# westi024/RadTxfr

Measured on AMD Instinct MI355X. Metric: wavenumber*layer points/s (32-layer TUD, 500-6000 cm^-1 @ 0.001 cm^-1), higher is better.
Workload: dtype f32; 1 GPU; C3: 32-layer TUD (tau,Lu,Ld) StandardAtmosphere rows 1-32, 500-6000 cm^-1 @ 0.001 cm^-1; n_wavenumbers=5500000, n_layers=32, n_lines=100000, n_angles=30, line_table=synthetic HITRAN-format H2O+CO2, seed 20261005, parallelism=wavenumber-sharded x1, pipelines_per_gpu=3

## Files before the change

### include/radtxfr_hip.h

```cpp
#ifndef RADTXFR_HIP_H
#define RADTXFR_HIP_H

#include <stdint.h>

#ifdef __cplusplus
extern "C" {
#endif

#define RTX_VERSION 100

typedef struct rtx_grid {
  double xmin;
  double xmax;
  double step;
  int64_t n_total;
  int64_t offset;
  int64_t n;
} rtx_grid;

int rtx_version(void);
const char* rtx_last_error(void);
int rtx_device_info(char* name_h, int len, int* n_cu_h);

typedef struct rtx_lines rtx_lines;
// ... 40 lines not shown
                       const double* mass_h, double dil_air, double dil_self, double omega_wing, double omega_wing_hw,
                       double intensity_threshold, double scale, int profile, void* stream);

#define RTX_MAX_DILUENTS 8
int rtx_line_prep_mix(rtx_prep* prep, const rtx_lines* lines, const rtx_grid* grid, int n_layers, const double* T_h,
                      const double* p_atm_h, const double* qratio_h, const double* weight_h, const double* mass_h,
                      int n_dil, const int32_t* dil_h, const double* frac_h, double omega_wing, double omega_wing_hw,
                      double intensity_threshold, double scale, int profile, void* stream);
int rtx_line_prep_axis_mix(rtx_prep* prep, const rtx_lines* lines, const double* X_h, int64_t nx, int n_layers,
                           const double* T_h, const double* p_atm_h, const double* qratio_h, const double* weight_h,
                           const double* mass_h, int n_dil, const int32_t* dil_h, const double* frac_h, double omega_wing,
                           double omega_wing_hw, double intensity_threshold, double scale, int profile, void* stream);

int rtx_voigt_tile_points(void);
int rtx_voigt_sum(const rtx_prep* prep, const rtx_grid* grid, int n_layers, float* out_f32,
                  double* out_f64, int64_t ld, void* stream);
int rtx_voigt_sum_axis(const rtx_prep* prep, int n_layers, float* out_f32, double* out_f64, int64_t ld, void* stream);

int rtx_line_prep_dt(rtx_prep* prep, const rtx_lines* lines, const rtx_grid* grid, int n_layers, const double* T_h,
                     const double* p_atm_h, const double* qratio_h, const double* weight_h, const double* mass_h,
                     const double* dlnsw_h, double dil_air, double dil_self, double omega_wing, double omega_wing_hw,
                     double intensity_threshold, double scale, void* stream);
int rtx_voigt_sum_dt(const rtx_prep* prep, const rtx_grid* grid, int n_layers, float* out_f32, double* out_f64,
                     int64_t ld, void* stream);

int rtx_planck(const rtx_grid* grid, const double* X, int64_t nx, const double* T, int64_t nT,
               int wavelength, double* out, void* stream);

int rtx_brightness_temperature(const double* X, int64_t nx, const double* L, int64_t m,
                               int wavelength, double bad_value, double* T_out, void* stream);
int rtx_bt2l(const double* X, int64_t nx, const double* T, int64_t m, int wavelength,
             double bad_value, double* L_out, void* stream);

int rtx_tud(const float* OD, int64_t ld, const rtx_grid* grid, int n_layers, const double* T_h,
            int n_alt, const uint8_t* mask_h, int n_mu, const double* mu_h, int n_down,
            int n_angle, int return_od, float* tau, float* Lu, float* Ld, float* Ld_angles,
            int64_t ld_out, void* stream);
#define RTX_TUD_OD_NONNEG 1u
int rtx_tud_opts(const float* OD, int64_t ld, const rtx_grid* grid, int n_layers, const double* T_h,
                 int n_alt, const uint8_t* mask_h, int n_mu, const double* mu_h, int n_down,
                 int n_angle, int return_od, float* tau, float* Lu, float* Ld, float* Ld_angles,
                 int64_t ld_out, void* stream, unsigned flags);

int rtx_tud_jacobian(const float* OD, const float* OD_plus, const float* OD_minus, int64_t ld, double fd_step,
                     const float* K, int n_spec, const float* tau, int64_t ld_tau, const rtx_grid* grid,
                     int n_layers, const double* T_h, int n_alt, const uint8_t* mask_h, double mu, int n_down,
                     int n_angle, int return_od, const int32_t* layers_h, int n_lay, int t_pos, float* J,
                     int64_t ld_J, void* stream);
int rtx_tud_vjp(const float* OD, const float* OD_plus, const float* OD_minus, int64_t ld, double fd_step,
                const float* K, int n_spec, const float* tau, int64_t ld_tau, const rtx_grid* grid, int n_layers,
                const double* T_h, int n_alt, const uint8_t* mask_h, double mu, int n_down, int n_angle,
                int return_od, const int32_t* layers_h, int n_lay, int t_pos, const float* G_tau,
                const float* G_Lu, const float* G_Ld, int64_t ld_G, int n_vec, double* out, void* stream);
int rtx_tud_vjp_max_vectors(void);
int rtx_tud_jacobian_dod(const float* OD, const float* dOD_dT, int64_t ld, const float* K, int n_spec, const float* tau,
                         int64_t ld_tau, const rtx_grid* grid, int n_layers, const double* T_h, int n_alt,
                         const uint8_t* mask_h, double mu, int n_down, int n_angle, int return_od,
                         const int32_t* layers_h, int n_lay, int t_pos, float* J, int64_t ld_J, void* stream);
int rtx_tud_vjp_dod(const float* OD, const float* dOD_dT, int64_t ld, const float* K, int n_spec, const float* tau,
                    int64_t ld_tau, const rtx_grid* grid, int n_layers, const double* T_h, int n_alt,
                    const uint8_t* mask_h, double mu, int n_down, int n_angle, int return_od, const int32_t* layers_h,
                    int n_lay, int t_pos, const float* G_tau, const float* G_Lu, const float* G_Ld, int64_t ld_G,
                    int n_vec, double* out, void* stream);
int rtx_tud_jvp(const float* OD, const float* OD_plus, const float* OD_minus, int64_t ld, double fd_step,
                const float* K, int n_spec, const float* tau, int64_t ld_tau, const rtx_grid* grid, int n_layers,
                const double* T_h, int n_alt, const uint8_t* mask_h, double mu, int n_down, int n_angle,
                int return_od, int t_pos, const double* V_h, int n_vec, float* d_tau, float* d_Lu, float* d_Ld,
                int64_t ld_out, void* stream);
int rtx_tud_jvp_dod(const float* OD, const float* dOD_dT, int64_t ld, const float* K, int n_spec, const float* tau,
                    int64_t ld_tau, const rtx_grid* grid, int n_layers, const double* T_h, int n_alt,
                    const uint8_t* mask_h, double mu, int n_down, int n_angle, int return_od, int t_pos,
                    const double* V_h, int n_vec, float* d_tau, float* d_Lu, float* d_Ld, int64_t ld_out, void* stream);
int rtx_tud_jvp_max_vectors(void);
int rtx_tud_gtable_size(void);
int rtx_tud_gtable(int n_angle, double* table_h, double* g0_h);

int rtx_compute_tud(rtx_prep* prep, const rtx_lines* lines, const rtx_grid* grid, int n_layers,
                    const double* T_h, const double* p_atm_h, const double* qratio_h,
                    const double* weight_h, const double* mass_h, double dil_air, double dil_self,
                    double omega_wing, double omega_wing_hw, double intensity_threshold, int n_alt,
                    const uint8_t* mask_h, int n_mu, const double* mu_h, int n_down, int n_angle,
                    int return_od, float* OD, int64_t ld_od, float* tau, float* Lu, float* Ld,
                    int64_t ld_out, void* stream);

int rtx_apparent_radiance(const double* X, int64_t nX, const float* emis, int64_t nE,
                          const double* Ts, int64_t nA, const float* tau, const float* La,
                          const float* Ld, const double* dT, int64_t nT, float* L, float* Ls,
                          void* stream);

int rtx_ils(int kind, const rtx_grid* grid, const double* X, int64_t nx, const float* Y,
            int64_t nS, int64_t ldY, int nB, const double* centre, const double* sigma,
            float* Y_out, void* stream);

int rtx_srf_apply(const rtx_grid* grid, const double* X, int64_t nx, const float* Y, int64_t nS,
                  int64_t ldY, int nB, const int32_t* knot_start, const double* knot_x,
                  const float* knot_r, float* Y_out, float* wsum_out, void* stream);
int rtx_srf_chunk_points(void);
int rtx_srf_max_knots(void);

int rtx_interp_knots(const rtx_grid* grid, const double* X, int64_t nx, const double* Xk,
                     int64_t nk, const float* F, int64_t nS, float* out, void* stream);

int rtx_band_moments(int kind, const rtx_grid* grid, const float* tau, const float* La,
                     const float* Ld, double Ts, const double* Xk, int64_t nk, int nB,
                     const double* centre, const double* sigma, float* N_out, float* C_out,
                     float* M_out, int32_t* jrange_out, void* stream);
int rtx_band_mix(const float* N, const float* C, const float* M, const int32_t* jrange, int nB,
                 int64_t nk, const float* E, int64_t nE, float* out, void* stream);

int rtx_srf_moments(const rtx_grid* grid, const float* tau, const float* La, const float* Ld,
                    const double* Ts_h, int nT, const double* Xk, int64_t nk, int nB,
                    const int32_t* knot_start, const double* knot_x, const float* knot_r,
                    float* N_out, float* C_out, float* M_out, int32_t* jrange_out, void* stream);
int rtx_srf_moments_max_temps(void);

int rtx_srf_radiance_vjp(const rtx_grid* grid, const float* tau, const float* La, const float* Ld,
                         const double* Ts_h, int nT, const double* Xk, int64_t nk, int nB,
                         const int32_t* knot_start, const double* knot_x, const float* knot_r,
                         const float* E, int64_t nE, const float* g, float* G_tau, float* G_La,
                         float* G_Ld, double* dTs, double* dE, void* stream);
int rtx_srf_norms(const rtx_grid* grid, int nB, const int32_t* knot_start, const double* knot_x,
                  const float* knot_r, float* N_out, void* stream);

int rtx_srf_radiance_jvp(const rtx_grid* grid, const float* tau, const float* Ld, const float* d_tau,
                         const float* d_La, const float* d_Ld, int64_t ld_d, const double* Ts_h,
                         const double* dTs_h, int nT, const double* Xk, int64_t nk, int nB,
                         const int32_t* knot_start, const double* knot_x, const float* knot_r,
                         const float* N, const float* M, const int32_t* jrange, const float* E,
                         const float* dE, int64_t nE, int n_vec, float* dL, void* stream);
int rtx_srf_radiance_jvp_max_vectors(void);
int rtx_srf_radiance_jvp_max_temps(void);

int rtx_band_basis_moments(int kind, const rtx_grid* grid, const float* tau, const float* La,
                           const float* Ld, const double* Xk, int64_t nk, int nB,
                           const double* centre, const double* sigma, int Q,
                           const float* basis_coef_h, double node_span, float* N_out,
                           float* C_out, float* MLd_out, float* MB_out, int32_t* jrange_out,
                           void* stream);
int rtx_band_mix_stacked(const float* M, const int32_t* jrange, int nB, int n_stack, int64_t nk,
                         const float* E, int64_t nE, float* tab, void* stream);
int rtx_pixel_cube(int nB, int Q, const double* centre, const double* sigma, double node_span,
                   const float* s_node_h, const float* N, const float* C, const float* tab,
                   int nEnd, int64_t nPix, int nMix, const int32_t* kidx, const float* frac,
                   const double* Tpix, float* cube, void* stream);

int rtx_srf_cube_max_nodes(void);
int rtx_srf_cube_tables(const float* M, const int32_t* jrange, int nB, int Q, int64_t nk,
                        const float* E, int64_t nEnd, float* tab, void* stream);
int rtx_srf_pixel_cube(int nB, int Q, const double* T_node_h, const float* N, const float* C,
                       const float* tab, int nEnd, int64_t nPix, int nMix, const int32_t* kidx,
                       const float* frac, const double* Tpix, float* cube, void* stream);

int rtx_srf_pixel_cube_vjp(int nB, int Q, const double* T_node_h, const float* N, const float* tab,
                           int nEnd, int64_t nPix, int nMix, const int32_t* kidx, const float* frac,
                           const double* Tpix, const float* g, double* dT, double* dfrac, float* gL,
                           void* stream, unsigned flags);

int rtx_sdvoigt_sum(const rtx_prep* prep, const rtx_grid* grid, int n_layers, float* out_f32,
                    double* out_f64, int64_t ld, void* stream);

#define RTX_LS_PCQSDHC 0
#define RTX_LS_LORENTZ 1
#define RTX_LS_DOPPLER 2
#define RTX_CPF_HUM1_WEI 0
#define RTX_CPF_CPF3 1
int rtx_profile_eval(int kind, int64_t n_lines, const double* params, const double* sg, int64_t n,
// ... 75 lines not shown
```

### radtxfr_amd/_lib.py

```python
import ctypes as C
import os

_HERE = os.path.dirname(os.path.abspath(__file__))
LIB_PATH = os.environ.get("RADTXFR_LIB") or os.path.join(_HERE, "libradtxfr_hip.so")


class RtxGrid(C.Structure):
    _fields_ = [("xmin", C.c_double), ("xmax", C.c_double), ("step", C.c_double),
                ("n_total", C.c_int64), ("offset", C.c_int64), ("n", C.c_int64)]


_vp, _i64, _i32, _dbl = C.c_void_p, C.c_int64, C.c_int, C.c_double
_pd = C.POINTER(C.c_double)
_gp = C.POINTER(RtxGrid)

PROTOTYPES = {
    "rtx_version": (_i32, []),
    "rtx_last_error": (C.c_char_p, []),
    "rtx_device_info": (_i32, [C.c_char_p, _i32, C.POINTER(_i32)]),
    "rtx_lines_create": (_i32, [_i64, _i32] + [_vp] * 10 + [_vp, C.POINTER(_vp)]),
    "rtx_lines_free": (_i32, [_vp]),
    "rtx_lines_count": (_i64, [_vp]),
    "rtx_prep_create": (_i32, [_vp, _i32, _i64, C.POINTER(_vp)]),
    "rtx_prep_free": (_i32, [_vp]),
    "rtx_line_prep": (_i32, [_vp, _vp, _gp, _i32, _vp, _vp, _vp, _vp, _vp, _dbl, _dbl, _dbl, _dbl, _dbl, _dbl, _vp]),
    "rtx_line_prep_profile": (_i32, [_vp, _vp, _gp, _i32, _vp, _vp, _vp, _vp, _vp, _dbl, _dbl, _dbl, _dbl, _dbl, _dbl, _i32, _vp]),
    "rtx_prep_split_bound": (_i64, [_vp]),
    "rtx_line_prep_window": (_i32, [_vp, _vp, _gp, _i32, _vp, _vp, _vp, _vp, _vp, _vp, _dbl, _dbl, _dbl, _dbl, _dbl, _dbl, _i32, _vp]),
    "rtx_line_prep_axis": (_i32, [_vp, _vp, _vp, _i64, _i32, _vp, _vp, _vp, _vp, _vp, _dbl, _dbl, _dbl, _dbl, _dbl, _dbl, _i32, _vp]),
    "rtx_voigt_sum": (_i32, [_vp, _gp, _i32, _vp, _vp, _i64, _vp]),
    "rtx_voigt_sum_axis": (_i32, [_vp, _i32, _vp, _vp, _i64, _vp]),
    "rtx_sdvoigt_sum": (_i32, [_vp, _gp, _i32, _vp, _vp, _i64, _vp]),
    "rtx_lines_set_sd": (_i32, [_vp, _vp, _vp]),
    "rtx_lines_set_deltap_self": (_i32, [_vp, _vp]),
    "rtx_lines_set_broadeners": (_i32, [_vp, _i32, _vp, _vp, _vp, _vp, _vp]),
    "rtx_line_prep_mix": (_i32, [_vp, _vp, _gp, _i32, _vp, _vp, _vp, _vp, _vp, _i32, _vp, _vp, _dbl, _dbl, _dbl, _dbl, _i32, _vp]),
    "rtx_line_prep_axis_mix": (_i32, [_vp, _vp, _vp, _i64, _i32, _vp, _vp, _vp, _vp, _vp, _i32, _vp, _vp, _dbl, _dbl, _dbl, _dbl,
                                       _i32, _vp]),
    "rtx_voigt_tile_points": (_i32, []),
    "rtx_planck": (_i32, [_gp, _vp, _i64, _vp, _i64, _i32, _vp, _vp]),
    "rtx_tud": (_i32, [_vp, _i64, _gp, _i32, _vp, _i32, _vp, _i32, _vp, _i32, _i32, _i32, _vp, _vp, _vp, _vp, _i64, _vp]),
    "rtx_tud_opts": (_i32, [_vp, _i64, _gp, _i32, _vp, _i32, _vp, _i32, _vp, _i32, _i32, _i32, _vp, _vp, _vp, _vp, _i64, _vp, C.c_uint]),
    "rtx_tud_jacobian": (_i32, [_vp, _vp, _vp, _i64, _dbl, _vp, _i32, _vp, _i64, _gp, _i32, _vp, _i32, _vp, _dbl, _i32, _i32,
                                 _i32, _vp, _i32, _i32, _vp, _i64, _vp]),
    "rtx_tud_vjp": (_i32, [_vp, _vp, _vp, _i64, _dbl, _vp, _i32, _vp, _i64, _gp, _i32, _vp, _i32, _vp, _dbl, _i32, _i32,
                            _i32, _vp, _i32, _i32, _vp, _vp, _vp, _i64, _i32, _vp, _vp]),
    "rtx_tud_vjp_max_vectors": (_i32, []),
    "rtx_line_prep_dt": (_i32, [_vp, _vp, _gp, _i32, _vp, _vp, _vp, _vp, _vp, _vp, _dbl, _dbl, _dbl, _dbl, _dbl, _dbl, _vp]),
    "rtx_voigt_sum_dt": (_i32, [_vp, _gp, _i32, _vp, _vp, _i64, _vp]),
    "rtx_tud_jacobian_dod": (_i32, [_vp, _vp, _i64, _vp, _i32, _vp, _i64, _gp, _i32, _vp, _i32, _vp, _dbl, _i32, _i32,
                                     _i32, _vp, _i32, _i32, _vp, _i64, _vp]),
    "rtx_tud_vjp_dod": (_i32, [_vp, _vp, _i64, _vp, _i32, _vp, _i64, _gp, _i32, _vp, _i32, _vp, _dbl, _i32, _i32,
                                _i32, _vp, _i32, _i32, _vp, _vp, _vp, _i64, _i32, _vp, _vp]),
    "rtx_tud_jvp": (_i32, [_vp, _vp, _vp, _i64, _dbl, _vp, _i32, _vp, _i64, _gp, _i32, _vp, _i32, _vp, _dbl, _i32, _i32,
                            _i32, _i32, _vp, _i32, _vp, _vp, _vp, _i64, _vp]),
    "rtx_tud_jvp_dod": (_i32, [_vp, _vp, _i64, _vp, _i32, _vp, _i64, _gp, _i32, _vp, _i32, _vp, _dbl, _i32, _i32,
                                _i32, _i32, _vp, _i32, _vp, _vp, _vp, _i64, _vp]),
    "rtx_tud_jvp_max_vectors": (_i32, []),
    "rtx_tud_gtable_size": (_i32, []),
    "rtx_tud_gtable": (_i32, [_i32, _vp, _vp]),
    "rtx_compute_tud": (_i32, [_vp, _vp, _gp, _i32, _vp, _vp, _vp, _vp, _vp, _dbl, _dbl, _dbl, _dbl, _dbl, _i32, _vp, _i32, _vp,
                                _i32, _i32, _i32, _vp, _i64, _vp, _vp, _vp, _i64, _vp]),
    "rtx_apparent_radiance": (_i32, [_vp, _i64, _vp, _i64, _vp, _i64, _vp, _vp, _vp, _vp, _i64, _vp, _vp, _vp]),
    "rtx_ils": (_i32, [_i32, _gp, _vp, _i64, _vp, _i64, _i64, _i32, _vp, _vp, _vp, _vp]),
    "rtx_srf_apply": (_i32, [_gp, _vp, _i64, _vp, _i64, _i64, _i32, _vp, _vp, _vp, _vp, _vp, _vp]),
    "rtx_srf_chunk_points": (_i32, []),
    "rtx_srf_max_knots": (_i32, []),
    "rtx_srf_moments": (_i32, [_gp, _vp, _vp, _vp, _vp, _i32, _vp, _i64, _i32, _vp, _vp, _vp, _vp, _vp, _vp, _vp, _vp]),
    "rtx_srf_moments_max_temps": (_i32, []),
    "rtx_srf_radiance_vjp": (_i32, [_gp, _vp, _vp, _vp, _vp, _i32, _vp, _i64, _i32, _vp, _vp, _vp, _vp, _i64, _vp, _vp, _vp, _vp,
                                     _vp, _vp, _vp]),
    "rtx_srf_norms": (_i32, [_gp, _i32, _vp, _vp, _vp, _vp, _vp]),
    "rtx_srf_radiance_jvp": (_i32, [_gp, _vp, _vp, _vp, _vp, _vp, _i64, _vp, _vp, _i32, _vp, _i64, _i32, _vp, _vp, _vp, _vp, _vp,
                                     _vp, _vp, _vp, _i64, _i32, _vp, _vp]),
    "rtx_srf_radiance_jvp_max_vectors": (_i32, []),
    "rtx_srf_radiance_jvp_max_temps": (_i32, []),
    "rtx_interp_knots": (_i32, [_gp, _vp, _i64, _vp, _i64, _vp, _i64, _vp, _vp]),
    "rtx_band_moments": (_i32, [_i32, _gp, _vp, _vp, _vp, _dbl, _vp, _i64, _i32, _vp, _vp, _vp, _vp, _vp, _vp, _vp]),
    "rtx_band_mix": (_i32, [_vp, _vp, _vp, _vp, _i32, _i64, _vp, _i64, _vp, _vp]),
    "rtx_band_basis_moments": (_i32, [_i32, _gp, _vp, _vp, _vp, _vp, _i64, _i32, _vp, _vp, _i32, _vp, _dbl,
                                      _vp, _vp, _vp, _vp, _vp, _vp]),
    "rtx_band_mix_stacked": (_i32, [_vp, _vp, _i32, _i32, _i64, _vp, _i64, _vp, _vp]),
    "rtx_pixel_cube": (_i32, [_i32, _i32, _vp, _vp, _dbl, _vp, _vp, _vp, _vp, _i32, _i64, _i32, _vp, _vp, _vp, _vp, _vp]),
    "rtx_srf_cube_max_nodes": (_i32, []),
    "rtx_srf_cube_tables": (_i32, [_vp, _vp, _i32, _i32, _i64, _vp, _i64, _vp, _vp]),
    "rtx_srf_pixel_cube": (_i32, [_i32, _i32, _vp, _vp, _vp, _vp, _i32, _i64, _i32, _vp, _vp, _vp, _vp, _vp]),
    "rtx_srf_pixel_cube_vjp": (_i32, [_i32, _i32, _vp, _vp, _vp, _i32, _i64, _i32, _vp, _vp, _vp, _vp, _vp, _vp, _vp, _vp, C.c_uint]),
    "rtx_fir_reflect": (_i32, [_vp, _i32, _i64, _i32, _i64, _vp, _i32, _i32, _vp, _i64, _vp]),
    "rtx_cubic_resample": (_i32, [_vp, _i64, _i32, _i64, _dbl, _dbl, _vp, _i64, _vp, _i64, _vp]),
    "rtx_cubic_end": (_i32, [_vp, _i64, _i32, _i64, _i32, _i32, _i32, _vp, _vp, _i64, _vp, _i64, _vp]),
    "rtx_cubic_resample_unchecked": (_i32, [_vp, _i64, _i32, _i64, _dbl, _dbl, _vp, _i64, _vp, _i64, _vp]),
    "rtx_hapi_spectrum": (_i32, [_i32, _gp, _vp, _vp, _i32, _i32, _i64, _i64, _dbl, _dbl, _vp, _i64, _vp]),
    "rtx_fir_same": (_i32, [_vp, _i32, _i64, _i32, _i64, _vp, _i64, _dbl, _i64, _i64, _vp, _i64, _vp]),
    "rtx_profile_eval": (_i32, [_i32, _i64, _vp, _vp, _i64, _vp, _vp, _i64, _vp]),
    "rtx_profile_sum": (_i32, [_i64, _vp, _vp, _vp, _vp, _i64, _vp, _vp]),
    "rtx_cpf_eval": (_i32, [_i32, _vp, _vp, _i64, _vp, _vp, _vp]),
    "rtx_lines_set_ht": (_i32, [_vp, _i32, _vp, _vp]),
    "rtx_ht_create": (_i32, [_i64, _i32, _i64, C.POINTER(_vp)]),
    "rtx_ht_free": (_i32, [_vp]),
    "rtx_ht_prep": (_i32, [_vp, _vp, _vp, _i64, _i32, _vp, _vp, _vp, _vp, _vp, _i32, _vp, _vp, _dbl, _dbl, _dbl, _dbl, _vp]),
    "rtx_ht_sum": (_i32, [_vp, _i32, _vp, _vp, _i64, _vp]),
    "rtx_ht_params": (_i32, [_vp, _i32, _vp, _vp, _vp, _vp]),
    "rtx_fir_tile_points": (_i32, []),
    "rtx_fir_chunk_taps": (_i32, []),
    "rtx_brightness_temperature": (_i32, [_vp, _i64, _vp, _i64, _i32, _dbl, _vp, _vp]),
    "rtx_bt2l": (_i32, [_vp, _i64, _vp, _i64, _i32, _dbl, _vp, _vp]),
    "rtx_xs_lut_create": (_i32, [_i32, _i64, _i64, C.POINTER(_vp)]),
    "rtx_xs_lut_free": (_i32, [_vp]),
    "rtx_xs_lut_bytes": (_i64, [_vp]),
    "rtx_xs_lut_set_rows": (_i32, [_vp, _i64, _i64, _vp, _vp]),
    "rtx_xs_lut_get_rows": (_i32, [_vp, _i64, _i64, _vp, _vp]),
    "rtx_xs_od": (_i32, [_vp, _i64, _i64, _i32, _vp, _vp, _vp, _i64, _vp]),
    "rtx_xs_tile_points": (_i32, []),
    "rtx_xs_od_d": (_i32, [_vp, _i64, _i64, _i32, _vp, _vp, _i32, _vp, _vp, _vp, _vp, _i64, _vp, C.c_uint]),
    "rtx_continuum_add": (_i32, [_gp, _i32, _vp, _i32, _vp, _vp, _vp, _vp, _i64, _vp, _i64, _vp, C.c_uint]),
    "rtx_continuum_tile_points": (_i32, []),
    "rtx_continuum_add_d": (_i32, [_gp, _i32, _vp, _i32, _vp, _vp, _vp, _vp, _vp, _vp, _i64, _vp, _i32, _vp, _vp, _i64, _vp,
                                   C.c_uint]),
    "rtx_comm_init_all": (_i32, [_i32, _vp, _i32, C.POINTER(_vp)]),
    "rtx_comm_backend": (_i32, [_vp]),
    "rtx_allgather": (_i32, [_vp, _vp, _vp, _i64, _vp]),
    "rtx_comm_destroy": (_i32, [_vp]),
}

_lib = None


class RtxError(RuntimeError):
    pass


def load():
    global _lib
    if _lib is not None:
        return _lib
    if not os.path.exists(LIB_PATH):
        raise RtxError(
            f"{LIB_PATH} not found: build it with `python -c 'import __graft_entry__ as g; g.build()'` "
            f"or `make -C radtxfr_amd/csrc` (hipcc --offload-arch=gfx950). There is no CPU fallback.")
    import torch
    lib = C.CDLL(LIB_PATH)
    for name, (res, args) in PROTOTYPES.items():
        try:
            fn = getattr(lib, name)
        except AttributeError as e:
# ... 19 lines not shown
```

### radtxfr_amd/csrc/rtx_common.h

```cpp
#pragma once
#include <hip/hip_runtime.h>
#include <math.h>
#include <stdint.h>
#include <stdio.h>

#include <vector>

#include "../../include/radtxfr_hip.h"
#include "rtx_devmem.h"

void rtx_set_error(const char* fmt, ...);
#define RTX_FAIL(...)          \
  do {                         \
    rtx_set_error(__VA_ARGS__); \
    return 1;                  \
  } while (0)
#define RTX_HIP(call)                                                                        \
  do {                                                                                       \
    hipError_t e_ = (call);                                                                  \
    if (e_ != hipSuccess) RTX_FAIL("%s:%d %s -> %s", __FILE__, __LINE__, #call, hipGetErrorString(e_)); \
  } while (0)
#define RTX_LAUNCH_CHECK()                                                                   \
  do {                                                                                       \
    hipError_t e_ = hipGetLastError();                                                       \
// ... 69 lines not shown
  double nu, cte, Gam0, Shift0, Gam2, WS;
  double inv_Gam2, csqrtY;
};

struct __attribute__((aligned(16))) LineRecDT64 {
  double alpha;
  double sx;
  double gy;
  double h;
};
struct __attribute__((aligned(16))) LineRecDT {
  float alpha, sx, yp, h;
  float Ap;
  float yh;
  float y2;
  float y;
};

struct rtx_lines {
  long long n = 0;
  int n_species = 0;
  DevBuf<double> nu, sw, elower, gamma_air, gamma_self, n_air, n_self, delta_air, deltap_air, delta_self;
  DevBuf<double> sd_air, sd_self;
  DevBuf<double> deltap_self;
  DevBuf<double> zn;
  DevBuf<int> species;
  std::vector<double> nu_host;
  double ga_max = 0.0, gs_max = 0.0, n_lo = 1e300, n_hi = -1e300;
  double na_lo = 1e300, na_hi = -1e300, ns_lo = 1e300, ns_hi = -1e300;
  int n_extra = 0;
  DevBuf<double> x_gamma, x_n, x_delta, x_deltap, x_sd;
  std::vector<double> x_gmax, x_nlo, x_nhi;
  DevBuf<double> ht_data;
  DevBuf<const double*> ht_ptr;
};

#ifndef RTX_SPLIT_PART
#define RTX_SPLIT_PART 256
#endif
#ifndef RTX_SPLIT_MIN
#define RTX_SPLIT_MIN 768
#endif
struct __attribute__((aligned(16))) SplitItem {
  int tile, k;
  int lo, hi;
  int part;
  int extra;
  int pad0, pad1;
};

struct rtx_prep {
  long long n_lines = 0;
  int max_layers = 0;
  int n_layers = 0;
  DevBuf<LineRec> rec;
  DevBuf<LineRec64> rec64;
  DevBuf<int> ic;
  DevBuf<int2> win;
  DevBuf<int> maxhw;
  int* smally = nullptr;
  int* n_items = nullptr;
  DevBuf<int2> ranges;
  DevBuf<LineRecSD> recsd;
  long long max_tiles = 0;
  DevBuf<double> env;
  double scale = 0.0;
  DevBuf<SplitItem> items;
  DevBuf<float> part_ws;
  long long split_bound = 0;
  double split_W = 0.0;
  double split_xmin = 0.0, split_step = 0.0;
  long long split_off = 0, split_n = 0;
  int split_layers = 0;
  const void* split_lines = nullptr;
  DevBuf<double> X;
  long long nx = 0;
  int axis = 0;
  DevBuf<double> twin;
  DevBuf<double> frac;
  DevBuf<LineRecDT> drec;
  DevBuf<LineRecDT64> drec64;
  DevBuf<double> dlnsw;
  int dT = 0;
};
```

### radtxfr_amd/csrc/rtx_tud.hip

```cpp
#include <math.h>
#include <stdlib.h>
#include <string.h>

#include <map>
#include <mutex>
#include <vector>

#include "rtx_tud_common.h"

struct PlanckArgs {
  GridDev g;
  const double* X;
  long long nx, nT;
  const double* T;
  int wavelength;
  double* out;
};

__global__ __launch_bounds__(256) void planck_kernel(PlanckArgs a) {
  const long long total = a.nx * a.nT;
  for (long long e = (long long)blockIdx.x * blockDim.x + threadIdx.x; e < total; e += (long long)gridDim.x * blockDim.x) {
    const long long i = e / a.nT, j = e - i * a.nT;
    double X = a.X ? a.X[i] : grid_x(a.g, a.g.offset + i);
    const double T = a.T[j];
// ... 47 lines not shown
    double X = a.X[i];
    const double v = a.in[e];
    double r;
    bool bad;
    if (a.inverse) {
      double L = v;
      if (a.wavelength) {
        X = X * 1e-6;  L = L * 1e4;
        r = RT_C2 / (X * log(1.0 + RT_C1 / (pow(X, 5.0) * L)));
      } else {
        X = X * 100.0;  L = L * 1e-4;
        r = RT_C2 * X / log(RT_C1 * (X * X * X) / L + 1.0);
      }
      bad = !isfinite(L) || (L <= 0.0);
    } else {
      const double T = v;
      if (a.wavelength) {
        X = X * 1e-6;
        r = RT_C1 / (pow(X, 5.0) * (exp(RT_C2 / (X * T)) - 1.0));
        r *= 1e-4;
      } else {
        X = X * 100.0;
        r = RT_C1 * (X * X * X) / (exp(RT_C2 * X / T) - 1.0);
        r *= 1e4;
      }
      bad = !isfinite(r) || (T <= 0.0);
    }
    a.out[e] = bad ? a.bad : r;
  }
}

static int launch_bt(const double* X, int64_t nx, const double* in, int64_t m, int wavelength, int inverse, double bad,
                     double* out, void* stream) {
  if (nx < 0 || m < 0) RTX_FAIL("negative size");
  if (nx == 0 || m == 0) return 0;
  if (!X || !in || !out) RTX_FAIL("a required pointer is NULL");
  BtArgs a;
  a.X = X; a.nx = nx; a.m = m; a.in = in; a.wavelength = wavelength; a.inverse = inverse; a.bad = bad; a.out = out;
  long long blocks = (nx * m + 255) / 256;
  if (blocks > 256 * 32) blocks = 256 * 32;
  hipLaunchKernelGGL(bt_kernel, dim3((unsigned)blocks), dim3(256), 0, (hipStream_t)stream, a);
  RTX_LAUNCH_CHECK();
  return 0;
}

extern "C" int rtx_brightness_temperature(const double* X, int64_t nx, const double* L, int64_t m, int wavelength,
                                          double bad_value, double* T_out, void* stream) {
  return launch_bt(X, nx, L, m, wavelength, 1, bad_value, T_out, stream);
}

extern "C" int rtx_bt2l(const double* X, int64_t nx, const double* T, int64_t m, int wavelength, double bad_value,
                        double* L_out, void* stream) {
  return launch_bt(X, nx, T, m, wavelength, 0, bad_value, L_out, stream);
}

#define TUD_MAX_LAYERS 128
#define TUD_MAX_ANGLES 128
#define TUD_MAX_ALT 16
#define TUD_MAX_MU 8

struct TudArgs {
  const float* OD;
  long long ld, ld_out;
  GridDev g;
  int n_layers, n_alt, n_mu, n_down, n_ang, return_od;
  float* tau;
  float* Lu;
  float* Ld;
  float* Ld_ang;
  int n_ang_real;
  float inv_wsum;
  double c2l2e_over_T[TUD_MAX_LAYERS];
  double c2l2e_over_Tmax, c2l2e_over_Tmin;
  float ang_c[TUD_MAX_ANGLES];
  float ang_w[TUD_MAX_ANGLES];
  float ang_cmin, ang_cmax;
  float mu_c[TUD_MAX_MU];
  float mu[TUD_MAX_MU];
  unsigned int mask[TUD_MAX_ALT][TUD_MAX_LAYERS / 32];
  int count[TUD_MAX_ALT];
  const double* gtab;
  double g0;
  int skip;
};

#define TUD_OPAQUE_Y 26.0f

__device__ __forceinline__ double readlane_f64(double v, int lane) {
  const int lo = __builtin_amdgcn_readlane(__double2loint(v), lane), hi = __builtin_amdgcn_readlane(__double2hiint(v), lane);
  return __hiloint2double(hi, lo);
}
struct TudLane {
  bool live;
  long long i;
  const float* __restrict__ od_col;
  double x, c1x3;
  double ct_a, ct_b;
  __device__ __forceinline__ explicit TudLane(const TudArgs& a) {
    const long long i_raw = (long long)blockIdx.x * blockDim.x + threadIdx.x;
    live = i_raw < a.g.n;
    i = live ? i_raw : a.g.n - 1;
    od_col = a.OD + i;
    x = grid_x(a.g, a.g.offset + i);
    const double x100 = x * 100.0;
    c1x3 = RT_C1 * (x100 * x100 * x100) * 1e4;
  }
  __device__ __forceinline__ void layer_consts(const TudArgs& a) {
    const int lane_id = threadIdx.x & 63, nL = a.n_layers;
    ct_a = a.c2l2e_over_T[lane_id < nL ? lane_id : 0];
    ct_b = a.c2l2e_over_T[lane_id + 64 < nL ? lane_id + 64 : 0];
  }
  __device__ __forceinline__ double c2l2e_of(int k) const { return readlane_f64(k < 64 ? ct_a : ct_b, k & 63); }
  __device__ __forceinline__ float planck(int k) const { return planck_f32(c1x3, x, c2l2e_of(k)); }
};

struct LayerMask {
  unsigned w0, w1, w2, w3;
  __device__ __forceinline__ bool bit(int k) const {
    const unsigned w = k < 32 ? w0 : k < 64 ? w1 : k < 96 ? w2 : w3;
    return (w >> (k & 31)) & 1u;
  }
};
__device__ __forceinline__ LayerMask layer_mask(const TudArgs& a, int ia) {
  return LayerMask{a.mask[ia][0], a.mask[ia][1], a.mask[ia][2], a.mask[ia][3]};
}

__device__ __forceinline__ float up_step(float Lu, float B, float y) {
  return (y > -TUD_THIN_Y) ? fmaf(em_thin(y), B - Lu, Lu) : fmaf(__builtin_amdgcn_exp2f(y), Lu - B, B);
}

__device__ __forceinline__ float opaque_y(const TudArgs& a, const TudLane& l) {
  const float b_hot = planck_f32(l.c1x3, l.x, a.c2l2e_over_Tmax), b_cold = planck_f32(l.c1x3, l.x, a.c2l2e_over_Tmin);
  const float r = __builtin_amdgcn_logf(b_hot / b_cold);
  return (b_cold > 0.f && r == r && r < 1e30f) ? TUD_OPAQUE_Y + 1.0f + fmaxf(r, 0.f) : 3.0e38f;
}

#ifndef TUD_STAGE
#define TUD_STAGE 4
#endif
#ifndef TUD_ABLATE
#define TUD_ABLATE 0
#endif
#ifndef TUD_ILP
#define TUD_ILP 8
#endif
#define TUD_COL_LAYERS 36
template <int NA, bool COL>
__global__ __launch_bounds__(256) void tud_kernel(TudArgs a) {
  extern __shared__ float s_od[];
  float (*s_stage)[256] = reinterpret_cast<float (*)[256]>(s_od);
  TudLane ln(a);
  const bool live = ln.live;
  const long long i = ln.i;
  const int nL = a.n_layers;
  const float* __restrict__ od_col = ln.od_col;
  if (COL) {
    float* dst = &s_stage[0][threadIdx.x & ~63u];
    for (int k = 0; k < nL; ++k)
      __builtin_amdgcn_global_load_lds((const __attribute__((address_space(1))) void*)(od_col + (size_t)k * a.ld),
                                       (__attribute__((address_space(3))) void*)(dst + k * 256), 4, 0, 0);
  }
  const double x = ln.x, c1x3 = ln.c1x3;
  if (COL) asm volatile("s_waitcnt vmcnt(0)" ::: "memory");
  ln.layer_consts(a);
  auto od_at = [&](int k) -> float { return COL ? s_stage[k][threadIdx.x] : od_col[(size_t)k * a.ld]; };
  auto planck_of = [&](int k) -> float { return COL ? planck_f32(c1x3, x, readlane_f64(ln.ct_a, k & 63)) : ln.planck(k); };
// ... 241 lines not shown
}

struct PlanckNodes {
  float c0, c1, c2;
  float c0b, c1b, c2b;
  float t;
};
__device__ __forceinline__ PlanckNodes planck_nodes_setup(const TudArgs& a, const TudLane& l) {
  PlanckNodes P;
  const double ct_a = l.ct_a, ct_b = l.ct_b;
  const int nL = a.n_layers;
  const long long i0w = (long long)blockIdx.x * blockDim.x + (threadIdx.x & ~63u);
  const float t1 = 32.0f / 63.0f;
  float b[3], bb[3];
#pragma unroll
  for (int n = 0; n < 3; ++n) {
    const double xn = grid_x(a.g, a.g.offset + i0w + (n == 0 ? 0 : n == 1 ? 32 : 63));
    const double x100 = xn * 100.0;
    const double c1x3 = RT_C1 * (x100 * x100 * x100) * 1e4;
    b[n] = planck_f32(c1x3, xn, ct_a);
    bb[n] = nL > 64 ? planck_f32(c1x3, xn, ct_b) : 0.f;
  }
  {
    const float d01 = (b[1] - b[0]) / t1, d12 = (b[2] - b[1]) / (1.0f - t1);
    P.c2 = d12 - d01; P.c1 = d01 - P.c2 * t1; P.c0 = b[0];
  }
  {
    const float d01 = (bb[1] - bb[0]) / t1, d12 = (bb[2] - bb[1]) / (1.0f - t1);
    P.c2b = d12 - d01; P.c1b = d01 - P.c2b * t1; P.c0b = bb[0];
  }
  P.t = (float)(threadIdx.x & 63) * (1.0f / 63.0f);
  return P;
}
__device__ __forceinline__ float planck_nodes_eval(const PlanckNodes& P, bool hi, int lane) {
  const float c0 = __int_as_float(__builtin_amdgcn_readlane(__float_as_int(hi ? P.c0b : P.c0), lane));
  const float c1 = __int_as_float(__builtin_amdgcn_readlane(__float_as_int(hi ? P.c1b : P.c1), lane));
  const float c2 = __int_as_float(__builtin_amdgcn_readlane(__float_as_int(hi ? P.c2b : P.c2), lane));
  return fmaf(fmaf(c2, P.t, c1), P.t, c0);
}
__device__ __forceinline__ float planck_nodes_eval(const PlanckNodes& P, int k) {
  if (k < 64) return planck_nodes_eval(P, false, k);
  return planck_nodes_eval(P, true, k - 64);
}

__device__ __forceinline__ void tudg_load(double* s_g, const TudArgs& a) {
  for (int t = threadIdx.x; t < TUDG_NINT * 4; t += 256) reinterpret_cast<double2*>(s_g)[t] = reinterpret_cast<const double2*>(a.gtab)[t];
}

struct TudDown {
  double S, g_prev, g_floor;
  float acc;
  bool live;
  __device__ __forceinline__ TudDown(const double* s_g, const TudArgs& a, const TudLane& l) {
    S = 0.0;
    g_prev = tudg_eval(s_g, 0.0);
    acc = 0.f;
    g_floor = a.g0 * (double)__builtin_amdgcn_exp2f(-fminf(opaque_y(a, l), 120.0f));
    live = a.n_down > 0;
  }
  __device__ __forceinline__ TudDown(const double* s_g, const TudArgs& a, float y_opq) {
    S = 0.0;
    g_prev = tudg_eval(s_g, 0.0);
    acc = 0.f;
    g_floor = a.g0 * (double)__builtin_amdgcn_exp2f(-fminf(y_opq, 120.0f));
    live = a.n_down > 0;
  }
  __device__ __forceinline__ void step(const double* s_g, float od, float B) {
    S += (double)od;
    const double g = tudg_eval(s_g, S);
    acc = fmaf(B, (float)(g_prev - g), acc);
    g_prev = g;
    if (__ballot(g > g_floor) == 0ull) live = false;
  }
  __device__ __forceinline__ float result(const TudArgs& a) const {
    return (S != S) ? __builtin_nanf("") : acc * a.inv_wsum;
  }
};

#define TUD_SKIP_SCAN (3 * TUD_STAGE)
#define TUD_SKIP_BOTTOM TUD_STAGE
#define TUD_SKIP_MARGIN 8.0f
#define TUD_SKIP_TAU0 151.0f

template <bool PN, bool SKIP>
__global__ __launch_bounds__(256) void tud_g_kernel(TudArgs a) {
  static_assert(PN || !SKIP, "the look at the top is written for the Planck-node instantiation");
  __shared__ double s_g[TUDG_NINT * 8];
  __shared__ float s_stage[(SKIP ? 2 : 1) * TUD_STAGE][256];
  tudg_load(s_g, a);
  TudLane ln(a);
  const int nL = a.n_layers;
  const float* __restrict__ od_col = ln.od_col;
  float nxt[TUD_STAGE];
#pragma unroll
  for (int t = 0; t < TUD_STAGE; ++t) nxt[t] = od_col[(size_t)(t < nL ? t : nL - 1) * a.ld];
  ln.layer_consts(a);
  const LayerMask mask0 = layer_mask(a, 0);
  PlanckNodes PNd;
  if (PN) PNd = planck_nodes_setup(a, ln);
  __syncthreads();

  for (int p = 1; p < a.n_alt * a.n_mu; ++p) {
    const int ia = p / a.n_mu, im = p - ia * a.n_mu;
    const int cnt = a.count[ia];
    const float c = a.mu_c[im];
    float s = 0.f, Lu = 0.f;
    for (int k = 0; k < nL; ++k) {
      const float od = ln.od_col[(size_t)k * a.ld];
      if ((a.mask[ia][k >> 5] >> (k & 31)) & 1u) s += od;
      if (k < cnt) Lu = up_step(Lu, PN ? planck_nodes_eval(PNd, k) : ln.planck(k), od * c);
    }
    if (ln.live) {
      const size_t o = (size_t)p * (size_t)a.ld_out + (size_t)ln.i;
      a.tau[o] = a.return_od ? s * a.mu[im] : __builtin_amdgcn_exp2f(s * c);
      a.Lu[o] = Lu;
    }
  }

  const int nd = a.n_down, cnt0 = a.count[0];
  const float c0 = a.mu_c[0];
  float s0 = 0.f, Lu0 = 0.f;
  const float y_opq = SKIP ? opaque_y(a, ln) : 0.f;
  TudDown down = SKIP ? TudDown(s_g, a, y_opq) : TudDown(s_g, a, ln);
  bool skip_armed = SKIP;
  const unsigned long long m_lo = (unsigned long long)mask0.w0 | ((unsigned long long)mask0.w1 << 32);
  const unsigned long long m_hi = (unsigned long long)mask0.w2 | ((unsigned long long)mask0.w3 << 32);
  const size_t bump = (size_t)TUD_STAGE * (size_t)a.ld;
  const float y_up = y_opq + TUD_SKIP_MARGIN;
  const int k_top = (cnt0 - 1) & ~(TUD_STAGE - 1);
  int k_look = -1;
  const float* pf[TUD_STAGE];
#pragma unroll
  for (int t = 0; t < TUD_STAGE; ++t) pf[t] = od_col + (size_t)(TUD_STAGE + t) * (size_t)a.ld;
  for (int kc = 0; kc < nL; kc += TUD_STAGE) {
#pragma unroll
    for (int t = 0; t < TUD_STAGE; ++t) s_stage[t][threadIdx.x] = nxt[t];
    if (kc + 2 * TUD_STAGE <= nL) {
#pragma unroll
      for (int t = 0; t < TUD_STAGE; ++t) nxt[t] = *pf[t];
    } else {
#pragma unroll
      for (int t = 0; t < TUD_STAGE; ++t)
        if (kc + TUD_STAGE + t < nL) nxt[t] = *pf[t];
    }
#pragma unroll
    for (int t = 0; t < TUD_STAGE; ++t) pf[t] += bump;
    const int k_hi = kc + TUD_STAGE < nL ? kc + TUD_STAGE : nL;
    if (PN && k_hi == kc + TUD_STAGE && k_hi <= cnt0 && k_hi <= nd) {
      const unsigned mchunk = (unsigned)((kc < 64 ? m_lo : m_hi) >> (kc & 63));
      const bool hi_set = kc >= 64;
#pragma unroll
      for (int t = 0; t < TUD_STAGE; ++t) {
        const float od = s_stage[t][threadIdx.x];
        if ((mchunk >> t) & 1u) s0 += od;
        const float B = planck_nodes_eval(PNd, hi_set, (kc & 63) + t);
        Lu0 = up_step(Lu0, B, od * c0);
        if (down.live) down.step(s_g, od, B);
      }
      if (SKIP && !down.live) {
        if (skip_armed) {
          skip_armed = false;
          if (k_hi <= TUD_SKIP_BOTTOM && k_hi + TUD_STAGE <= k_top) { k_look = k_hi; break; }
        }
      }
    } else {
      for (int k = kc; k < k_hi; ++k) {
        const float od = s_stage[k - kc][threadIdx.x];
        if (mask0.bit(k)) s0 += od;
        const bool up = k < cnt0, dn = down.live && k < nd;
        if (!up && !dn) continue;
        const float B = PN ? planck_nodes_eval(PNd, k) : ln.planck(k);
        if (up) Lu0 = up_step(Lu0, B, od * c0);
        if (dn) down.step(s_g, od, B);
      }
      if (SKIP && skip_armed && !(down.live && k_hi < nd)) {
        skip_armed = false;
        if (k_hi <= TUD_SKIP_BOTTOM && k_hi + TUD_STAGE <= k_top) { k_look = k_hi; break; }
      }
    }
  }
  if (SKIP && k_look >= 0) {
    int kc = k_look;
    unsigned tid_top = threadIdx.x;
    asm volatile("" : "+v"(tid_top));
    const long long i_top = (long long)blockIdx.x * blockDim.x + tid_top;
    const float* __restrict__ od_top = a.OD + (i_top < a.g.n ? i_top : a.g.n - 1);
    constexpr int NC = TUD_SKIP_SCAN / TUD_STAGE;
    const float ac0 = -c0;
    const int k_deep = k_top - (TUD_SKIP_SCAN - TUD_STAGE);
    const int k_scan = k_deep > kc + TUD_STAGE ? k_deep : kc + TUD_STAGE;
    static_assert(NC == 3, "the look at the top is laid out for three chunks");
    float v0[TUD_STAGE];
#pragma unroll
    for (int t = 0; t < TUD_STAGE; ++t) v0[t] = od_top[(size_t)(k_top + t < cnt0 ? k_top + t : cnt0 - 1) * (size_t)a.ld];
    {
      float* dst = &s_stage[0][threadIdx.x & ~63u];
      const int n_dma = k_top - 2 * TUD_STAGE >= k_scan ? 2 * TUD_STAGE : k_top - TUD_STAGE >= k_scan ? TUD_STAGE : 0;
      const float* pc = od_top + (size_t)(k_top - n_dma) * (size_t)a.ld;
      float* d = dst + (n_dma == TUD_STAGE ? TUD_STAGE * 256 : 0);
#pragma unroll 1
      for (int j = 0; j < n_dma; ++j) {
        __builtin_amdgcn_global_load_lds((const __attribute__((address_space(1))) void*)pc, (__attribute__((address_space(3))) void*)d, 4, 0, 0);
        pc += a.ld;
        d += 256;
      }
    }
    asm volatile("s_waitcnt vmcnt(0)" ::: "memory");
    float s_top = 0.f;
#pragma unroll
    for (int t = TUD_STAGE - 1; t >= 0; --t)
      if (k_top + t < cnt0) s_top += v0[t];
    int k_res = -1;
    if (__ballot(s_top * ac0 >= y_up) == ~0ull) k_res = k_top;
#pragma unroll 1
    for (int c = 1; c < NC && k_res < 0 && k_top - c * TUD_STAGE >= k_scan; ++c) {
      const int slot = c == 1 ? TUD_STAGE : 0;
#pragma unroll
      for (int t = TUD_STAGE - 1; t >= 0; --t) s_top += s_stage[slot + t][threadIdx.x];
      if (__ballot(s_top * ac0 >= y_up) == ~0ull) k_res = k_top - c * TUD_STAGE;
    }
    if (k_res < 0) {
#pragma unroll
      for (int t = 0; t < TUD_STAGE; ++t) pf[t] = od_top + (size_t)(kc + TUD_STAGE + t) * (size_t)a.ld;
      for (; kc < cnt0; kc += TUD_STAGE) {
#pragma unroll
        for (int t = 0; t < TUD_STAGE; ++t) s_stage[t][threadIdx.x] = nxt[t];
#pragma unroll
        for (int t = 0; t < TUD_STAGE; ++t)
          if (kc + TUD_STAGE + t < cnt0) nxt[t] = *pf[t];
#pragma unroll
        for (int t = 0; t < TUD_STAGE; ++t) pf[t] += bump;
        if (kc + TUD_STAGE <= cnt0) {
          const bool hi_set = kc >= 64;
#pragma unroll
          for (int t = 0; t < TUD_STAGE; ++t) {
            const float od = s_stage[t][threadIdx.x];
            s0 += od;
            Lu0 = up_step(Lu0, planck_nodes_eval(PNd, hi_set, (kc & 63) + t), od * c0);
          }
        } else {
          for (int k = kc; k < cnt0; ++k) {
            const float od = s_stage[k - kc][threadIdx.x];
            s0 += od;
            Lu0 = up_step(Lu0, planck_nodes_eval(PNd, k), od * c0);
          }
        }
      }
    } else {
    for (int km = kc; km < k_res; km += TUD_STAGE) {
      if (__ballot((s0 + s_top) * ac0 >= TUD_SKIP_TAU0) == ~0ull) break;
      float w[TUD_STAGE];
#pragma unroll
      for (int t = 0; t < TUD_STAGE; ++t) w[t] = od_top[(size_t)(km + t) * (size_t)a.ld];
#pragma unroll
      for (int t = 0; t < TUD_STAGE; ++t) s0 += w[t];
    }
#pragma unroll 1
    for (int kb = k_res; kb < k_top; kb += TUD_STAGE) {
      const int slot = kb == k_top - TUD_STAGE ? TUD_STAGE : 0;
#pragma unroll
      for (int t = 0; t < TUD_STAGE; ++t) {
        const float od = s_stage[slot + t][threadIdx.x];
        s0 += od;
        Lu0 = up_step(Lu0, planck_nodes_eval(PNd, kb + t), od * c0);
      }
    }
#pragma unroll
    for (int t = 0; t < TUD_STAGE; ++t) {
      if (k_top + t < cnt0) {
        s0 += v0[t];
        Lu0 = up_step(Lu0, planck_nodes_eval(PNd, k_top + t), v0[t] * c0);
      }
    }
    }
  }
  long long i_out = ln.i;
  bool live_out = ln.live;
  if (SKIP) {
    unsigned tid_out = threadIdx.x;
    asm volatile("" : "+v"(tid_out));
    i_out = (long long)blockIdx.x * blockDim.x + tid_out;
    live_out = i_out < a.g.n;
  }
  if (live_out) {
    a.tau[i_out] = a.return_od ? s0 * a.mu[0] : __builtin_amdgcn_exp2f(s0 * c0);
    a.Lu[i_out] = Lu0;
    a.Ld[i_out] = down.result(a);
  }
}

#ifndef TUDG_PB
#define TUDG_PB 3
#endif
template <int PB>
__global__ __launch_bounds__(256) void tud_g_pairs_kernel(TudArgs a) {
  __shared__ double s_g[TUDG_NINT * 8];
  __shared__ float s_stage[TUD_STAGE][256];
  tudg_load(s_g, a);
  TudLane ln(a);
  const int nL = a.n_layers;
  const float* __restrict__ od_col = ln.od_col;
  ln.layer_consts(a);
// ... 131 lines not shown
        s_run += od;
#pragma unroll
        for (int m = 0; m < NMU; ++m)
          if (NMU == 1 || m < n_mu) Lu[m] = up_step(Lu[m], B, od * cm[m]);
        if ((snap_chunk >> t) & 1u) snapshot(kc + t + 1);
        if (down.live) down.step(s_g, od, B);
      }
      continue;
    }
    for (int k = kc; k < k_hi; ++k) {
      const float od = s_stage[k - kc][threadIdx.x];
      const bool up = k < cnt_max, dn = down.live && k < nd;
      if (!up && !dn) continue;
      const float B = PN ? planck_nodes_eval(PNd, k) : ln.planck(k);
      if (up) {
        s_run += od;
#pragma unroll
        for (int m = 0; m < NMU; ++m)
          if (m < n_mu) Lu[m] = up_step(Lu[m], B, od * cm[m]);
        snapshot(k + 1);
      }
      if (dn) down.step(s_g, od, B);
    }
  }
  if (ln.live) a.Ld[ln.i] = down.result(a);
}

static void tudg_build(int n_angle, std::vector<double>& tab, double& g0_out) {
  const TudQuadrature quad = tud_quadrature(n_angle);
  std::vector<double> sec;
  for (int ii = 1; ii < n_angle; ++ii) sec.push_back(1.0 / cos(quad.th[ii]));
  auto G = [&](double S) { double r = 0.0; for (size_t q = 0; q < sec.size(); ++q) r += quad.w[q + 1] * exp(-S * sec[q]); return r; };
  constexpr int N = TUDG_DEG + 1;
  tab.assign((size_t)TUDG_NINT * 8, 0.0);
  for (int idx = 0; idx < TUDG_NINT; ++idx) {
    double lo, hi;
    if (idx < TUDG_NLOG) {
      union { int i; float f; } a0, a1;
      a0.i = (TUDG_BASE + idx) << (23 - TUDG_M);
      a1.i = (TUDG_BASE + idx + 1) << (23 - TUDG_M);
      lo = (double)a0.f - (double)TUDG_OFF;
      hi = (double)a1.f - (double)TUDG_OFF;
      if (lo < 0.0) lo = 0.0;
      if (hi > (double)TUDG_SWITCH) hi = (double)TUDG_SWITCH;
    } else {
      lo = (double)TUDG_SWITCH + 0.5 * (idx - TUDG_NLOG);
      hi = lo + 0.5;
    }
    const double mid = 0.5 * (lo + hi), hw = 0.5 * (hi - lo) * 1.002;
    double y[N], c[N];
    for (int k = 0; k < N; ++k) y[k] = G(mid + hw * cos(M_PI * (k + 0.5) / N));
    for (int j = 0; j < N; ++j) {
      double sacc = 0.0;
      for (int k = 0; k < N; ++k) sacc += y[k] * cos(M_PI * j * (k + 0.5) / N);
      c[j] = sacc * (j == 0 ? 1.0 : 2.0) / N;
    }
    double mono[N] = {0}, Tm[N] = {0}, Tc[N] = {0}, Tn[N];
    Tm[0] = 1.0;
    Tc[1] = 1.0;
    mono[0] += c[0];
    if (N > 1) mono[1] += c[1];
    for (int n = 2; n < N; ++n) {
      for (int d = 0; d < N; ++d) Tn[d] = (d > 0 ? 2.0 * Tc[d - 1] : 0.0) - Tm[d];
      for (int d = 0; d < N; ++d) { mono[d] += c[n] * Tn[d]; Tm[d] = Tc[d]; Tc[d] = Tn[d]; }
    }
    double* row = &tab[(size_t)idx * 8];
    row[0] = mid;
    double sc = 1.0;
    for (int d = 0; d < N; ++d) { row[1 + d] = mono[d] * sc; sc /= hw; }
  }
  g0_out = quad.wsum;
}

extern "C" int rtx_tud_gtable_size(void) { return TUDG_NINT * 8; }
extern "C" int rtx_tud_gtable(int n_angle, double* table_h, double* g0_h) {
  if (n_angle < 1 || n_angle > TUD_MAX_ANGLES - 32) RTX_FAIL("n_angle=%d outside [1,%d]", n_angle, TUD_MAX_ANGLES - 32);
  if (!table_h || !g0_h) RTX_FAIL("a required pointer is NULL");
  std::vector<double> tab;
  tudg_build(n_angle, tab, *g0_h);
  memcpy(table_h, tab.data(), tab.size() * sizeof(double));
  return 0;
}

static int tudg_table(int n_angle, DevTableCache<double>::Hit* out) {
  static DevTableCache<double>* const cache = new DevTableCache<double>(0);
  int dev = 0;
  RTX_HIP(hipGetDevice(&dev));
  return cache->get(dev, &n_angle, sizeof(n_angle), [&](std::vector<double>& tab) { double g0; tudg_build(n_angle, tab, g0); return 0; }, out);
}

static int tud_launch(void (*kernel)(TudArgs), const TudArgs& a, size_t lds_bytes, hipStream_t st) {
  hipLaunchKernelGGL(kernel, dim3((unsigned)((a.g.n + 255) / 256)), dim3(256), lds_bytes, st, a);
  RTX_LAUNCH_CHECK();
  return 0;
}

template <int NA>
static int launch_tud(TudArgs& a, int na, hipStream_t st) {
  const int na_pad = na == 0 ? NA : ((na + NA - 1) / NA) * NA;
  float cmin = (float)LOG2E, cmax = (float)LOG2E;
  for (int q = 0; q < na; ++q) { cmin = q == 0 ? -a.ang_c[q] : fminf(cmin, -a.ang_c[q]); cmax = q == 0 ? -a.ang_c[q] : fmaxf(cmax, -a.ang_c[q]); }
  for (int q = na; q < na_pad; ++q) { a.ang_c[q] = na > 0 ? a.ang_c[na - 1] : (float)(-LOG2E); a.ang_w[q] = 0.f; }
  a.ang_cmin = cmin; a.ang_cmax = cmax;
  a.n_ang = na_pad;
  if (a.n_layers <= TUD_COL_LAYERS) return tud_launch(tud_kernel<NA, true>, a, (size_t)a.n_layers * 256 * sizeof(float), st);
  return tud_launch(tud_kernel<NA, false>, a, (size_t)TUD_STAGE * 256 * sizeof(float), st);
}

extern "C" int rtx_tud_opts(const float* OD, int64_t ld, const rtx_grid* grid, int n_layers, const double* T_h, int n_alt,
                            const uint8_t* mask_h, int n_mu, const double* mu_h, int n_down, int n_angle, int return_od,
                            float* tau, float* Lu, float* Ld, float* Ld_angles, int64_t ld_out, void* stream, unsigned flags) {
  if (rtx_check_grid(grid)) return 1;
  if (flags & ~(unsigned)RTX_TUD_OD_NONNEG) RTX_FAIL("flags=0x%x: unknown bits", flags);
  if (!OD || !T_h || !mask_h || !mu_h || !tau || !Lu || !Ld) RTX_FAIL("a required pointer is NULL");
  if (n_layers < 1 || n_layers > TUD_MAX_LAYERS) RTX_FAIL("n_layers=%d outside [1,%d]", n_layers, TUD_MAX_LAYERS);
  if (n_alt < 1 || n_alt > TUD_MAX_ALT) RTX_FAIL("n_alt=%d outside [1,%d]", n_alt, TUD_MAX_ALT);
  if (n_mu < 1 || n_mu > TUD_MAX_MU) RTX_FAIL("n_mu=%d outside [1,%d]", n_mu, TUD_MAX_MU);
  if (n_angle < 1 || n_angle > TUD_MAX_ANGLES - 32) RTX_FAIL("n_angle=%d outside [1,%d]", n_angle, TUD_MAX_ANGLES - 32);
  if (n_down < 0 || n_down > n_layers) RTX_FAIL("n_down=%d outside [0,%d]", n_down, n_layers);
  if (ld < grid->n || ld_out < grid->n) RTX_FAIL("leading dimension smaller than the shard");
  if (grid->n == 0) return 0;
  TudArgs a;
  memset(&a, 0, sizeof(a));
  a.OD = OD; a.ld = ld; a.ld_out = ld_out; a.g = to_dev(grid);
  a.n_layers = n_layers; a.n_alt = n_alt; a.n_mu = n_mu; a.n_down = n_down; a.return_od = return_od;
  a.tau = tau; a.Lu = Lu; a.Ld = Ld; a.Ld_ang = Ld_angles;
  if (tud_layer_consts(T_h, n_layers, a.c2l2e_over_T)) return 1;
  double t_max = T_h[0], t_min = T_h[0];
  for (int k = 1; k < n_layers; ++k) {
    if (T_h[k] > t_max) t_max = T_h[k];
    if (T_h[k] < t_min) t_min = T_h[k];
  }
  a.c2l2e_over_Tmax = c2l2e_over(t_max);
  a.c2l2e_over_Tmin = c2l2e_over(t_min);
  for (int ia = 0; ia < n_alt; ++ia) {
    int c = 0;
    for (int k = 0; k < n_layers; ++k)
      if (mask_h[(size_t)ia * n_layers + k]) { a.mask[ia][k >> 5] |= 1u << (k & 31); ++c; }
    a.count[ia] = c;
  }
  for (int m = 0; m < n_mu; ++m) { a.mu[m] = (float)mu_h[m]; a.mu_c[m] = (float)(-LOG2E * mu_h[m]); }
  const TudQuadrature quad = tud_quadrature(n_angle);
  int na = 0;
  for (int ii = Ld_angles ? 0 : 1; ii < n_angle; ++ii) {
    a.ang_c[na] = (float)(-LOG2E / cos(quad.th[ii]));
    a.ang_w[na] = (float)quad.w[ii];
    ++na;
  }
  a.n_ang_real = na;
  a.inv_wsum = (float)(1.0 / quad.wsum);
  if (na == 0) a.inv_wsum = NAN;
  hipStream_t st = (hipStream_t)stream;
  static int force_streams = -1;
  if (force_streams < 0) { const char* e = getenv("RADTXFR_TUD_KERNEL"); force_streams = (e && !strcmp(e, "streams")) ? 1 : 0; }
  if (!Ld_angles && !force_streams) {
    DevTableCache<double>::Hit gt;
    if (tudg_table(n_angle, &gt)) return 1;
    a.gtab = gt.d; a.g0 = quad.wsum;
    bool prefix = true;
    for (int ia = 0; ia < n_alt && prefix; ++ia)
      for (int k = 0; k < n_layers; ++k)
        if ((mask_h[(size_t)ia * n_layers + k] != 0) != (k < a.count[ia])) { prefix = false; break; }
    const double nu_lo = grid->xmin;
    const bool pn = nu_lo > 0.0 && (4.0 / nu_lo + RT_C2 * 100.0 / t_min) * 63.0 * grid->step <= 7e-3;
    void (*kernel)(TudArgs);
    if (n_alt * n_mu == 1) {
      kernel = pn ? tud_g_kernel<true, false> : tud_g_kernel<false, false>;
      static int skip_on = -1;
      if (skip_on < 0) { const char* e = getenv("RADTXFR_TUD_SKIP"); skip_on = (e && !strcmp(e, "0")) ? 0 : 1; }
      a.skip = skip_on && (flags & RTX_TUD_OD_NONNEG) && !return_od && prefix && pn;
      if (a.skip) kernel = tud_g_kernel<true, true>;
    }
    else if (prefix && n_mu == 1) kernel = pn ? tud_g_snap_kernel<1, true> : tud_g_snap_kernel<1, false>;
    else if (prefix) kernel = pn ? tud_g_snap_kernel<TUD_MAX_MU, true> : tud_g_snap_kernel<TUD_MAX_MU, false>;
    else kernel = tud_g_pairs_kernel<TUDG_PB>;
    return tud_launch(kernel, a, 0, st);
  }
  if (na <= 4) return launch_tud<4>(a, na, st);
  if (na <= 8) return launch_tud<8>(a, na, st);
  if (na <= 16) return launch_tud<16>(a, na, st);
  if (na <= 24) return launch_tud<24>(a, na, st);
  if (na <= 29) return launch_tud<29>(a, na, st);
  return launch_tud<32>(a, na, st);
}

extern "C" int rtx_tud(const float* OD, int64_t ld, const rtx_grid* grid, int n_layers, const double* T_h, int n_alt,
                       const uint8_t* mask_h, int n_mu, const double* mu_h, int n_down, int n_angle, int return_od,
                       float* tau, float* Lu, float* Ld, float* Ld_angles, int64_t ld_out, void* stream) {
  return rtx_tud_opts(OD, ld, grid, n_layers, T_h, n_alt, mask_h, n_mu, mu_h, n_down, n_angle, return_od, tau, Lu, Ld, Ld_angles,
                      ld_out, stream, 0u);
}

extern "C" int rtx_compute_tud(rtx_prep* prep, const rtx_lines* lines, const rtx_grid* grid, int n_layers, const double* T_h,
                               const double* p_atm_h, const double* qratio_h, const double* weight_h, const double* mass_h,
                               double dil_air, double dil_self, double omega_wing, double omega_wing_hw,
                               double intensity_threshold, int n_alt, const uint8_t* mask_h, int n_mu, const double* mu_h,
                               int n_down, int n_angle, int return_od, float* OD, int64_t ld_od, float* tau, float* Lu,
                               float* Ld, int64_t ld_out, void* stream) {
  if (!OD) RTX_FAIL("OD workspace is NULL");
  if (rtx_line_prep_profile(prep, lines, grid, n_layers, T_h, p_atm_h, qratio_h, weight_h, mass_h, dil_air, dil_self, omega_wing,
                            omega_wing_hw, intensity_threshold, 1.0, RTX_PROFILE_VOIGT, stream))
    return 1;
  if (rtx_voigt_sum(prep, grid, n_layers, OD, nullptr, ld_od, stream)) return 1;
  auto nonneg = [](const double* v, long long n) {
    for (long long j = 0; j < n; ++j)
      if (!(v[j] >= 0.0 && v[j] <= 1.7976931348623157e308)) return false;
    return true;
  };
  const long long n_sl = (long long)lines->n_species * n_layers;
  const unsigned flags = nonneg(weight_h, n_sl) && nonneg(qratio_h, n_sl) && nonneg(T_h, n_layers) && nonneg(p_atm_h, n_layers)
                             ? RTX_TUD_OD_NONNEG : 0u;
  return rtx_tud_opts(OD, ld_od, grid, n_layers, T_h, n_alt, mask_h, n_mu, mu_h, n_down, n_angle, return_od, tau, Lu, Ld, nullptr,
                      ld_out, stream, flags);
}
```

### radtxfr_amd/csrc/rtx_voigt.hip

```cpp
#include <stdlib.h>
#include <string.h>

#include "rtx_common.h"

#include "rtx_voigt_math.h"

struct RangeArgs {
  const int* ic;
  const int* maxhw;
  const int2* win;
  long long n_lines;
  int n_tiles, tile, n_layers, n_steps;
  long long n;
  int2* ranges;
  SplitItem* items;
  int* n_items;
  long long items_cap;
};

#define RNG_G 16
__device__ __forceinline__ unsigned group_bits(unsigned long long b, int lane) { return (unsigned)(b >> (lane & 48)) & 0xffffu; }

template <bool STRICT>
__device__ __forceinline__ void bound_step(const int* __restrict__ ic, int& lo, int& hi, int v, int sub, int lane) {
  const unsigned width = (unsigned)(hi - lo);
  const int stride = (int)((width + RNG_G) / (unsigned)(RNG_G + 1));
  const long long pl = (long long)lo + (long long)(sub + 1) * stride - 1;
  const bool inside = width > 0 && pl < (long long)hi;
  const int p = inside ? (int)pl : lo;
  const bool pred = inside && (STRICT ? ic[p] < v : ic[p] <= v);
  const int c = __popc(group_bits(__ballot(pred), lane));
  if (width > 0) {
    const long long cap = (long long)lo + (long long)(c + 1) * stride - 1;
    if (c < RNG_G && cap < (long long)hi) hi = (int)cap;
    lo += c * stride;
  }
}

__global__ __launch_bounds__(256) void tile_ranges_kernel(RangeArgs a) {
  const int lane = threadIdx.x & 63, sub = lane & (RNG_G - 1);
  const int t = (int)((blockIdx.x * blockDim.x + threadIdx.x) / RNG_G);
  const int k = blockIdx.y;
  const bool live = t < a.n_tiles;
  const long long ia = (long long)t * a.tile;
  long long ib = ia + a.tile;
  if (ib > a.n) ib = a.n;
  const long long hw = a.maxhw[k];
  int l0 = 0, h0 = live ? (int)a.n_lines : 0, l1 = 0, h1 = h0;
  {
    const long long v0 = ia - hw, v1 = ib - 1 + hw;
    const int k0 = (int)(v0 < -2147483647LL ? -2147483647LL : v0), k1 = (int)(v1 > 2147483647LL ? 2147483647LL : v1);
    for (int it = 0; it < a.n_steps; ++it) {
      bound_step<true>(a.ic, l0, h0, k0, sub, lane);
      bound_step<false>(a.ic, l1, h1, k1, sub, lane);
    }
  }
  if (l1 < l0) l1 = l0;
  const int2* __restrict__ win = a.win + (size_t)k * (size_t)a.n_lines;
  long long first = l1, last = l1;
  {
    int base = l0, top = l1;
    bool done_f = base >= l1, done_b = done_f;
    while (__ballot(!done_f || !done_b)) {
      const int sf = base + sub, sb = top - 1 - sub;
      int2 wf = make_int2(0, 0), wb = wf;
      if (!done_f && sf < l1) wf = win[sf];
      if (!done_b && sb >= l0) wb = win[sb];
      const bool rf = (long long)wf.y > ia && (long long)wf.x < ib && wf.y > wf.x;
      const bool rb = (long long)wb.y > ia && (long long)wb.x < ib && wb.y > wb.x;
      const unsigned mf = group_bits(__ballot(rf), lane), mb = group_bits(__ballot(rb), lane);
      if (!done_f) {
        if (mf) { first = base + __builtin_ctz(mf); done_f = true; }
        else { base += RNG_G; done_f = base >= l1; }
      }
      if (!done_b) {
        if (mb) { last = top - __builtin_ctz(mb); done_b = true; }
        else { top -= RNG_G; done_b = top <= l0; }
      }
    }
    if (first >= l1) last = first = l1;
  }
  if (live && sub == 0) {
    const long long cnt = last - first;
    if (a.items && cnt > RTX_SPLIT_MIN) {
      const int extra = (int)((cnt - 1) / RTX_SPLIT_PART);
      const long long at = (long long)atomicAdd(a.n_items, extra);
      if (at + extra <= a.items_cap) {
        for (int p = 1; p <= extra; ++p) {
          SplitItem it;
          it.tile = t; it.k = k; it.part = p; it.extra = extra; it.pad0 = it.pad1 = 0;
          it.lo = (int)(first + (long long)p * RTX_SPLIT_PART);
          const long long e = first + (long long)(p + 1) * RTX_SPLIT_PART;
          it.hi = (int)(e < last ? e : last);
          a.items[at + p - 1] = it;
        }
        last = first + RTX_SPLIT_PART;
      }
    }
    a.ranges[(size_t)k * a.n_tiles + t] = make_int2((int)first, (int)last);
  }
}

int rtx_voigt_scatter_tile_points(void);
extern "C" int rtx_voigt_tile_points(void) { return rtx_voigt_scatter_tile_points(); }

int rtx_voigt_sum_scatter(const rtx_prep* P, const rtx_grid* grid, int n_layers, float* out_f32, double* out_f64, int64_t ld,
                          hipStream_t st, void (*launch_ranges)(const rtx_prep*, const rtx_grid*, int, int, int, hipStream_t, int),
                          int nodal);

static void launch_tile_ranges(const rtx_prep* P, const rtx_grid* grid, int n_layers, int n_tiles, int tile, hipStream_t st, int split) {
  RangeArgs ra;
  const bool cut = split && P->split_bound > 0 && P->items.get();
  ra.items = cut ? P->items.get() : nullptr; ra.n_items = P->n_items; ra.items_cap = (long long)P->items.cap();
  ra.ic = P->ic.get(); ra.maxhw = P->maxhw.get(); ra.win = P->win.get(); ra.n_lines = P->n_lines; ra.n_tiles = n_tiles; ra.tile = tile;
  ra.n_layers = n_layers; ra.n = grid->n; ra.ranges = P->ranges.get();
  int n_steps = 1;
  for (long long w = P->n_lines; w > 0; w /= (RNG_G + 1)) ++n_steps;
  ra.n_steps = n_steps;
  hipLaunchKernelGGL(tile_ranges_kernel, dim3((n_tiles * RNG_G + 255) / 256, n_layers), dim3(256), 0, st, ra);
}

void rtx_launch_tile_ranges_n(const rtx_prep* P, long long n, int n_layers, int n_tiles, int tile, hipStream_t st) {
  rtx_grid g;
  memset(&g, 0, sizeof(g));
  g.n = n;
  launch_tile_ranges(P, &g, n_layers, n_tiles, tile, st, 0);
}

static int voigt_kernel_choice() {
  static int cached = -1;
  if (cached < 0) {
    const char* e = getenv("RADTXFR_VOIGT_KERNEL");
    cached = (e && strcmp(e, "scatter") == 0) ? 1 : 0;
  }
  return cached;
}

extern "C" int rtx_voigt_sum(const rtx_prep* P, const rtx_grid* grid, int n_layers, float* out_f32, double* out_f64,
                             int64_t ld, void* stream) {
  if (!P) RTX_FAIL("prep is NULL");
  if (P->axis) RTX_FAIL("the last prologue was rtx_line_prep_axis: sum with rtx_voigt_sum_axis");
  if (rtx_check_grid(grid)) return 1;
  if (n_layers < 1 || n_layers != P->n_layers) RTX_FAIL("n_layers=%d does not match the last rtx_line_prep (%d)", n_layers, P->n_layers);
  if (!out_f32 && !out_f64) RTX_FAIL("both outputs are NULL");
  if (ld < grid->n) RTX_FAIL("ld=%lld < n=%lld", (long long)ld, (long long)grid->n);
  if (grid->n == 0) return 0;
  hipStream_t st = (hipStream_t)stream;
  if (P->n_lines == 0) {
    if (out_f32) RTX_HIP(hipMemset2DAsync(out_f32, ld * sizeof(float), 0, grid->n * sizeof(float), n_layers, st));
    if (out_f64) RTX_HIP(hipMemset2DAsync(out_f64, ld * sizeof(double), 0, grid->n * sizeof(double), n_layers, st));
    return 0;
  }
  return rtx_voigt_sum_scatter(P, grid, n_layers, out_f32, out_f64, ld, st, launch_tile_ranges, voigt_kernel_choice() == 0);
}
```

### radtxfr_amd/csrc/rtx_voigt_scatter.hip

```cpp
#include "rtx_common.h"

#include "rtx_voigt_math.h"

#include "cheb8_64.inc"
#include "cheb16_tile.inc"
#include <vector>

#ifndef RTX_SC_ABLATE
#define RTX_SC_ABLATE 0
#endif
#ifndef RTX_SC_ASYM
#define RTX_SC_ASYM 1
#endif
#ifndef RTX_SC_OUTER
#define RTX_SC_OUTER 1
#endif
#ifndef RTX_SC_ROWS
#define RTX_SC_ROWS 16
#endif
#ifndef RTX_SC_NEAR
#define RTX_SC_NEAR 2
#endif
static_assert(RTX_SC_ROWS <= 31, "row masks are 32-bit");

#ifndef RTX_SC_STAMP
#define RTX_SC_STAMP 0
#endif
#define SC_NSTAMP 8
#define STAMP(i_)                                 \
  if (RTX_SC_STAMP) {                             \
    const long long t_now_ = (long long)clock64(); \
    t_ph[i_] += t_now_ - t_prev;                  \
    t_prev = t_now_;                              \
  }
struct ScArgs {
  unsigned long long* stamp;
  const LineRec* rec;
  const LineRec64* rec64;
  const int2* ranges;
  const int* smally;
  long long n_lines;
  int n_tiles;
  int tiles_per_xcd;
  GridDev g;
  float* out32;
  double* out64;
  long long ld;
  double inv_scale;
  const SplitItem* items;
  const int* n_items;
  float* part_ws;
};

struct RowGeom {
  int r_lo, r_hi;
  int c0, c1;
  int z0, z1;
  int n0, n1;
  bool part_l, part_r;
};
__device__ __forceinline__ RowGeom row_geom(int qi0, int qlo, int qhi, int qzw, int ia, int nt) {
  constexpr int ROWS = RTX_SC_ROWS;
  RowGeom g;
  const int dlo = qlo - ia, dhi = qhi - ia;
  const int lo_t = dlo > 0 ? dlo : 0, hi_t = dhi < nt ? dhi : nt;
  g.r_lo = lo_t >> 6;
  g.r_hi = (hi_t + 63) >> 6;
  g.c0 = (lo_t + 63) >> 6;
  g.c1 = dhi < nt ? hi_t >> 6 : g.r_hi;
  g.part_l = g.c0 != g.r_lo;
  g.part_r = g.c1 != g.r_hi;
  const int zw = qzw > 0 ? qzw : 0;
  const int zl = qi0 - zw - ia, zh = qi0 + zw - ia;
  g.z0 = ROWS;
  g.z1 = -1;
  if (qzw > 0 && zh >= 0 && zl < 64 * ROWS) {
    g.z0 = zl > 0 ? zl >> 6 : 0;
    g.z1 = (zh >> 6) < ROWS - 1 ? zh >> 6 : ROWS - 1;
  }
  const int rc = (qi0 - ia) >> 6;
  const int bl = zl >> 6, bh = zh >> 6;
  g.n0 = (rc - RTX_SC_NEAR) < bl ? rc - RTX_SC_NEAR : bl;
  g.n1 = (rc + RTX_SC_NEAR) > bh ? rc + RTX_SC_NEAR : bh;
  return g;
}

__device__ __forceinline__ int band_slot(int slot) { return slot; }
template <typename F>
__device__ __forceinline__ int band_slot(const F& slot) { return slot(); }
template <int MODE, bool CUT = true, int SER = -1, typename Slot>
__device__ __forceinline__ void band_row(const ScArgs& a, const LineRec64* __restrict__ rec64, const Slot& slot, const LineRec& q, float u, int i,
                                         float zw_f, float ulo, float uhi, bool small_y, float& num, float& rden, bool& touched) {
  constexpr bool CORE64 = MODE == 1;
  float x;
  farwing(u, q, x, num, rden);
  const bool in_band = fabsf(u) <= zw_f;
  const bool outer_row = MODE == 2 && small_y && RTX_SC_OUTER && __ballot(fabsf(x) < 5.5f) == 0ull;
  if (MODE == 2 && small_y && !outer_row) {
    const LineRec64 Q = rec64[band_slot(slot)];
    const double sg = grid_x(a.g, a.g.offset + (long long)i);
    const double x64 = -((Q.sg0 - sg) * Q.cte);
    if (fabs(x64) + Q.y < 15.0) {
      num = (float)(Q.A * weideman_re<double>(x64, Q.y));
      rden = 1.0f;
    }
  } else if (CORE64 ? small_y : (!small_y || outer_row)) {
    const float s32 = fabsf(x) + q.y;
    bool wz = s32 < 15.0f;
    const bool near = fabsf(s32 - 15.0f) < 2e-3f;
    if (CORE64 || __ballot(near)) {
      const LineRec64 Q = rec64[band_slot(slot)];
      const double sg = grid_x(a.g, a.g.offset + (long long)i);
      const double x64 = -((Q.sg0 - sg) * Q.cte);
      const bool wz64 = fabs(x64) + Q.y < 15.0;
      wz = (CORE64 || near) ? wz64 : wz;
      if (CORE64 && wz) {
        num = (float)(Q.A * weideman_re<double>(x64, Q.y));
        rden = 1.0f;
      }
    }
    if (!CORE64) {
      const bool series = RTX_SC_ASYM && (SER == 1 || (SER < 0 && q.y >= 6.0f) || __ballot(wz && fmaf(x, x, q.y * q.y) < 64.0f) == 0ull);
      if (wz) {
        if (MODE == 2 && outer_row) num = q.A * asymK_re<12>(x, q.y);
        else if (series) num = q.A * asym6_re(x, q.y);
        else num = q.A * weideman_re<float>(x, q.y);
        rden = 1.0f;
      }
    }
    if (CORE64) {
      num = in_band ? num : 0.f;
      touched = true;
    }
  } else {
    num = (CORE64 || in_band) ? 0.f : num;
// ... 119 lines not shown
template <bool CORE64>
__device__ __forceinline__ void scatter_tile(const ScArgs& a, float (*s_acc)[64 * RTX_SC_ROWS], int* s_touched, int b, int k) {
  constexpr int ROWS = RTX_SC_ROWS;
  constexpr int TILE = 64 * ROWS;
  const int tile = xcd_tile(b);
  if (tile >= a.n_tiles) return;
  const int wave = __builtin_amdgcn_readfirstlane((int)(threadIdx.x >> 6));
  const int lane = threadIdx.x & 63;
  const long long n = a.g.n;
  const int ia = tile * TILE;
  const int ib = (int)((long long)ia + TILE < n ? (long long)ia + TILE : n);
  const int nt = ib - ia;
  const LineRec* __restrict__ rec = a.rec + (size_t)k * (size_t)a.n_lines;
  const LineRec64* __restrict__ rec64 = a.rec64 + (size_t)k * (size_t)a.n_lines;
  const int2 rng = a.ranges[(size_t)k * a.n_tiles + tile];
  float* __restrict__ acc = s_acc[wave];
#pragma unroll
  for (int r = 0; r < ROWS; ++r) acc[r * 64 + lane] = 0.f;
  const float lanef = (float)lane;
  bool touched = false;

  for (int slot = rng.x + wave; slot < rng.y; slot += 4) visit_line<CORE64, false>(a, rec, rec64, slot, acc, ia, ib, nt, lane, lanef, touched);
  __syncthreads();

  if (CORE64) {
    if (threadIdx.x == 0) *s_touched = 0;
    __syncthreads();
    if (touched && lane == 0) *s_touched = 1;
    __syncthreads();
    if (!*s_touched) return;
  }
  store_tile<CORE64, false>(a, s_acc, nullptr, k, ia, ib, wave, lane);
}

template <bool CORE64>
__global__ __launch_bounds__(256) void voigt_scatter_kernel(ScArgs a) {
  __shared__ float s_acc[4][64 * RTX_SC_ROWS];
  __shared__ int s_touched;
  const int k = blockIdx.y;
  if (CORE64) {
    if (a.smally[k] == 0) return;
    for (int b = blockIdx.x; b < 8 * a.tiles_per_xcd; b += gridDim.x) {
      scatter_tile<true>(a, s_acc, &s_touched, b, k);
      __syncthreads();
    }
  } else {
    scatter_tile<false>(a, s_acc, &s_touched, blockIdx.x, k);
  }
}

#ifndef RTX_SC_WAVES
#define RTX_SC_WAVES 6
#endif
#ifndef SC_NW
#define SC_NW 2
#endif
#ifndef SC_EDGE_LIST
#define SC_EDGE_LIST 1
#endif
#ifndef SC_EDGE_CAP
#define SC_EDGE_CAP 32
#endif
#ifndef SC_EDGE_UNROLL
#define SC_EDGE_UNROLL 2
#endif
#ifndef RTX_SC_TILE_LEVEL
#define RTX_SC_TILE_LEVEL 1
#endif
#define RTX_SC_TILE_DIST 512
#ifndef RTX_SC_RED_REG
#define RTX_SC_RED_REG 1
#endif
#ifndef RTX_SC_MERGE
#define RTX_SC_MERGE 1
#endif
#ifndef RTX_SC_BAND_SPLIT
#define RTX_SC_BAND_SPLIT 1
#endif
#ifndef SC_ENT_CAP
#define SC_ENT_CAP (SC_EDGE_LIST ? 16 : 32)
#endif
template <bool SMALLY, bool PARTS = false>
__device__ __forceinline__ void nodal_tile(const ScArgs& a, const int b_or_tile, const int k, const int2 part_rng = make_int2(0, 0),
                                           float* __restrict__ part_out = nullptr) {
  constexpr int ROWS = RTX_SC_ROWS;
  constexpr int TILE = 64 * ROWS;
  __shared__ float s_acc[SC_NW][TILE];
  __shared__ float4 s_ent[SC_NW][SC_ENT_CAP][4];
  __shared__ float4 s_edge[SC_NW][SC_EDGE_LIST ? SC_EDGE_CAP : 1][2];
  __shared__ float s_nodsum[RTX_SC_ROWS][CHEB_N];
  static_assert((RTX_SC_ROWS * CHEB_N + TCHEB_N + 1) * 4 <= SC_ENT_CAP * 64, "row sums + tile sums fit in one wave's entry list");

  const int tile = part_out ? b_or_tile : xcd_tile(b_or_tile);
  if (tile >= a.n_tiles) return;
  const int wave = __builtin_amdgcn_readfirstlane((int)(threadIdx.x >> 6));
  const int lane = threadIdx.x & 63;
  const long long n = a.g.n;
  const int ia = tile * TILE;
  const int ib = (int)((long long)ia + TILE < n ? (long long)ia + TILE : n);
  const int nt = ib - ia;
  const LineRec* __restrict__ rec = a.rec + (size_t)k * (size_t)a.n_lines;
  const LineRec64* __restrict__ rec64 = a.rec64 + (size_t)k * (size_t)a.n_lines;
  const int2 rng = part_out ? part_rng : a.ranges[(size_t)k * a.n_tiles + tile];
  float* __restrict__ acc = s_acc[wave];
#pragma unroll
  for (int r = 0; r < ROWS; ++r) acc[r * 64 + lane] = 0.f;
  const float lanef = (float)lane;
  bool touched = false;
  long long t_ph[SC_NSTAMP] = {0, 0, 0, 0, 0, 0, 0, 0};
  long long t_prev = RTX_SC_STAMP ? (long long)clock64() : 0;
  const long long t_begin = t_prev;

  const int l = lane >> 3, j = lane & 7;
  float nod[ROWS];
#pragma unroll
  for (int r = 0; r < ROWS; ++r) nod[r] = 0.f;
  constexpr bool TILE_LEVEL = RTX_SC_TILE_LEVEL && ROWS == 16;
#ifndef RTX_SC_OFF_LDS
#define RTX_SC_OFF_LDS 0
#endif
#if !RTX_SC_OFF_LDS
  const float off_j = CHEB_OFF[j];
#endif
  if (lane < 8) {
    int lt = lane;
    if (SMALLY) asm volatile("" : "+v"(lt));
    s_nodsum[wave][lane] = CHEB_OFF[lt];
    if (TILE_LEVEL) s_nodsum[SC_NW + wave][lane] = TCHEB_OFF[lt];
  }
  float tnod_a = 0.f, tnod_b = 0.f;
  int n_tile_members = 0;
  int n_ent = 0;
  float4(*__restrict__ ent)[4] = s_ent[wave];
  auto below = [](unsigned long long m) -> int {
    return (int)__builtin_amdgcn_mbcnt_hi((unsigned)(m >> 32), __builtin_amdgcn_mbcnt_lo((unsigned)m, 0u));
  };
  auto pull = [](int src_lane, float v) -> float {
    return __int_as_float(__builtin_amdgcn_ds_bpermute(src_lane << 2, __float_as_int(v)));
  };

  static_assert(ROWS <= 16, "an entry packs its row masks as 16-bit halves");
  auto drain = [&]() {
    for (int e = 0; e < n_ent; ++e) {
      const float4 e0 = ent[e][0], e1 = ent[e][1], e2 = ent[e][2], e3 = ent[e][3];
      LineRec q;
      q.a = e0.x; q.c = e0.y; q.b1 = e0.z; q.b0 = e0.w;
      q.Ay = e1.x; q.Ay0 = e1.y; q.y = e1.z; q.A = e1.w;
      const float u0 = e2.x + lanef, ulo = e2.y, uhi = e2.z, zw_f = e2.w;
      const unsigned w0 = (unsigned)__builtin_amdgcn_readfirstlane(__float_as_int(e3.x));
      const unsigned w1 = (unsigned)__builtin_amdgcn_readfirstlane(__float_as_int(e3.y));
      unsigned m_pp = w0 & 0xffffu, m_ed = w0 >> 16, m_bd = w1 & 0xffffu, m_cut = w1 >> 16;
      auto slot = [&]() -> int { return __builtin_amdgcn_readfirstlane(__float_as_int(ent[e][3].z)); };
      STAMP(3);
      if (RTX_SC_ABLATE & 4) m_pp = m_ed = 0u;
      while (m_pp) {
        const int r = __builtin_ctz(m_pp);
        m_pp &= m_pp - 1u;
        float* p = acc + r * 64 + lane;
        float x0, n0, d0;
        farwing(u0 + (float)(64 * r), q, x0, n0, d0);
        p[0] = fmaf(n0, d0, p[0]);
      }
      while (m_ed) {
        const int r = __builtin_ctz(m_ed);
        m_ed &= m_ed - 1u;
        float* p = acc + r * 64 + lane;
        const float u = u0 + (float)(64 * r);
        float x0, n0, d0;
        farwing(u, q, x0, n0, d0);
        n0 = (u >= ulo && u < uhi) ? n0 : 0.f;
        p[0] = fmaf(n0, d0, p[0]);
      }
      STAMP(4);
      if (RTX_SC_ABLATE & 1) m_bd = m_cut = 0u;
      if (m_bd) {
        const unsigned fl = (unsigned)__builtin_amdgcn_readfirstlane(__float_as_int(ent[e][3].w));
        const bool small_y = fl & 1u, ser6 = fl & 2u;
        if (PARTS || !RTX_SC_BAND_SPLIT) m_cut = m_bd;
        const unsigned m_run = m_bd & ~m_cut;
        if (m_run) {
          int r = __builtin_ctz(m_run);
          const int r_end = r + __popc(m_run);
          if (ser6) {
            for (; r < r_end; ++r) {
              float* p = acc + r * 64 + lane;
              float num, rden;
              band_row<0, false, 1>(a, rec64, slot, q, u0 + (float)(64 * r), ia + 64 * r + lane, zw_f, ulo, uhi, false, num, rden, touched);
              p[0] = fmaf(num, rden, p[0]);
            }
          } else {
            for (; r < r_end; ++r) {
              float* p = acc + r * 64 + lane;
              float num, rden;
              band_row<0, false, 0>(a, rec64, slot, q, u0 + (float)(64 * r), ia + 64 * r + lane, zw_f, ulo, uhi, false, num, rden, touched);
              p[0] = fmaf(num, rden, p[0]);
            }
          }
        }
        while (m_cut) {
          const int r = __builtin_ctz(m_cut);
          m_cut &= m_cut - 1u;
          float* p = acc + r * 64 + lane;
          float num, rden;
          band_row<SMALLY ? 2 : 0>(a, rec64, slot, q, u0 + (float)(64 * r), ia + 64 * r + lane, zw_f, ulo, uhi, small_y, num, rden, touched);
          p[0] = fmaf(num, rden, p[0]);
        }
      }
      STAMP(5);
    }
    n_ent = 0;
  };

  int n_edge = 0;
  float4(*__restrict__ edg)[2] = s_edge[wave];
  auto edge_one = [&](const float4& E0, const float4& E1, int pk) {
    const int r = (pk >> 7) & 31, t = pk & 127;
    const bool right = (pk >> 12) & 1;
    float* p = acc + r * 64 + lane;
    const float u = E1.z + lanef;
    const float x = fmaf(u, E0.x, E0.y);
    const float xx = x * x;
    float num = fmaf(xx, E1.x, E1.y);
    const float rden = __builtin_amdgcn_rcpf(fmaf(xx + E0.z, xx, E0.w));
    const bool inside = (lane >= t) != right;
    num = inside ? num : 0.f;
    p[0] = fmaf(num, rden, p[0]);
  };
  auto drain_edges = [&]() {
    for (int e = 0; e < n_edge; e += SC_EDGE_UNROLL) {
      float4 E0[SC_EDGE_UNROLL], E1[SC_EDGE_UNROLL];
      int pk[SC_EDGE_UNROLL];
#pragma unroll
      for (int q = 0; q < SC_EDGE_UNROLL; ++q) {
        const int eq = e + q < n_edge ? e + q : e;
// ... 168 lines not shown
  drain();
  if (SC_EDGE_LIST) drain_edges();

  const int ln = (int)__builtin_amdgcn_mbcnt_hi(~0u, __builtin_amdgcn_mbcnt_lo(~0u, 0u));
#if RTX_SC_RED_REG
  auto ror8 = [](float v) -> float {
    return v + __int_as_float(__builtin_amdgcn_update_dpp(0, __float_as_int(v), 0x128, 0xf, 0xf, true));
  };
  auto swap16 = [](float a, float b) -> float {
    const auto s = __builtin_amdgcn_permlane16_swap((unsigned)__float_as_int(a), (unsigned)__float_as_int(b), false, false);
    return __int_as_float((int)s[0]) + __int_as_float((int)s[1]);
  };
  auto swap32 = [](float a, float b) -> float {
    const auto s = __builtin_amdgcn_permlane32_swap((unsigned)__float_as_int(a), (unsigned)__float_as_int(b), false, false);
    return __int_as_float((int)s[0]) + __int_as_float((int)s[1]);
  };
  static_assert(ROWS % 4 == 0, "the register reduction takes the tile rows four at a time");
#pragma unroll
  for (int q = 0; q < ROWS / 4; ++q) {
    const float v = swap32(swap16(ror8(nod[4 * q]), ror8(nod[4 * q + 1])), swap16(ror8(nod[4 * q + 2]), ror8(nod[4 * q + 3])));
    if (!(ln & 8)) reinterpret_cast<float*>(&s_ent[wave][0][0])[(4 * q + (ln >> 4)) * CHEB_N + (ln & 7)] = v;
  }
  if (TILE_LEVEL) {
    const float h = swap16(ror8(tnod_a), ror8(tnod_b));
    const float v = swap32(h, h);
    float* ts = reinterpret_cast<float*>(&s_ent[wave][0][0]) + ROWS * CHEB_N;
    if (ln < 8) ts[ln] = v;
    if ((ln & ~7) == 16) ts[15 - (ln & 7)] = v;
    if (ln == 0) ts[16] = __int_as_float(n_tile_members);
  }
#else
#pragma unroll
  for (int r = 0; r < ROWS; ++r) {
    float v = nod[r];
    v += __shfl_xor(v, 8);
    v += __shfl_xor(v, 16);
    v += __shfl_xor(v, 32);
    if (lane < 8) reinterpret_cast<float*>(&s_ent[wave][0][0])[r * CHEB_N + lane] = v;
  }
  if (TILE_LEVEL) {
    float va = tnod_a, vb = tnod_b;
    va += __shfl_xor(va, 8);  vb += __shfl_xor(vb, 8);
    va += __shfl_xor(va, 16); vb += __shfl_xor(vb, 16);
    va += __shfl_xor(va, 32); vb += __shfl_xor(vb, 32);
    float* ts = reinterpret_cast<float*>(&s_ent[wave][0][0]) + ROWS * CHEB_N;
    if (lane < 8) { ts[lane] = va; ts[15 - lane] = vb; }
    if (lane == 0) ts[16] = __int_as_float(n_tile_members);
  }
#endif
  STAMP(2);
  __syncthreads();
  STAMP(6);
  static_assert(SC_NW == 1 || SC_NW == 2 || SC_NW == 4, "one, two or four waves per workgroup");
  for (int o = wave * 64 + ln; o < ROWS * CHEB_N; o += 64 * SC_NW) {
    float v = reinterpret_cast<const float*>(&s_ent[0][0][0])[o];
    if constexpr (SC_NW >= 2) v += reinterpret_cast<const float*>(&s_ent[1][0][0])[o];
    if constexpr (SC_NW == 4) v += reinterpret_cast<const float*>(&s_ent[2][0][0])[o] + reinterpret_cast<const float*>(&s_ent[3][0][0])[o];
    if (TILE_LEVEL) {
      int any = 0;
#pragma unroll
      for (int w = 0; w < SC_NW; ++w) any |= __float_as_int(reinterpret_cast<const float*>(&s_ent[w][0][0])[ROWS * CHEB_N + 16]);
      if (any) {
        float c = 0.f;
#pragma unroll
        for (int t = 0; t < TCHEB_N; ++t) {
          float tsum = reinterpret_cast<const float*>(&s_ent[0][0][0])[ROWS * CHEB_N + t];
          if constexpr (SC_NW >= 2) tsum += reinterpret_cast<const float*>(&s_ent[1][0][0])[ROWS * CHEB_N + t];
          if constexpr (SC_NW == 4)
            tsum += reinterpret_cast<const float*>(&s_ent[2][0][0])[ROWS * CHEB_N + t] + reinterpret_cast<const float*>(&s_ent[3][0][0])[ROWS * CHEB_N + t];
          c = fmaf(TCHEB_M[t][o], tsum, c);
        }
        v += c;
      }
    }
    s_nodsum[o >> 3][o & 7] = v;
  }
  __syncthreads();
  {
    float wl[CHEB_N];
#pragma unroll
    for (int jj = 0; jj < CHEB_N; ++jj) wl[jj] = CHEB_W[lane][jj];
#pragma unroll 4
    for (int r = wave; r < ROWS; r += SC_NW) {
      const int t = r * 64 + lane;
      const long long i = (long long)ia + t;
      float f = 0.f;
#pragma unroll
      for (int jj = 0; jj < CHEB_N; ++jj) f = fmaf(wl[jj], s_nodsum[r][jj], f);
      float pp = s_acc[0][t];
      if constexpr (SC_NW >= 2) pp += s_acc[1][t];
      if constexpr (SC_NW == 4) pp += s_acc[2][t] + s_acc[3][t];
      const float v = pp + f;
      if (part_out) {
        part_out[t] = v;
      } else if (i < (long long)ib) {
        const size_t o = (size_t)k * (size_t)a.ld + (size_t)i;
        if (a.out32) a.out32[o] = v;
        if (a.out64) a.out64[o] = (double)v * a.inv_scale;
      }
    }
  }
  if (RTX_SC_STAMP && !part_out) {
    t_ph[7] = (long long)clock64() - t_begin;
    if (lane == 0) {
      unsigned long long* o = a.stamp + ((size_t)(blockIdx.y * gridDim.x + blockIdx.x) * SC_NW + wave) * SC_NSTAMP;
      for (int i = 0; i < SC_NSTAMP; ++i) o[i] = (unsigned long long)t_ph[i];
    }
  }
}

#ifndef RTX_SC_WAVES_SMALLY
#define RTX_SC_WAVES_SMALLY 4
#endif
template <bool SMALLY>
__global__ __launch_bounds__(64 * SC_NW, SMALLY ? RTX_SC_WAVES_SMALLY : RTX_SC_WAVES) void voigt_nodal_kernel(ScArgs a) {
  const int k = blockIdx.y;
  if ((a.smally[k] != 0) != SMALLY) return;
  if (SMALLY) {
    for (int b = blockIdx.x; b < 8 * a.tiles_per_xcd; b += gridDim.x) {
      nodal_tile<true>(a, b, k);
      __syncthreads();
    }
  } else {
    nodal_tile<false>(a, blockIdx.x, k);
  }
}

template <bool SMALLY>
__global__ __launch_bounds__(64 * SC_NW, SMALLY ? RTX_SC_WAVES_SMALLY : RTX_SC_WAVES) void voigt_nodal_parts_kernel(ScArgs a) {
  const int i = blockIdx.x;
  if (i >= *a.n_items) return;
  const SplitItem it = a.items[i];
  if ((a.smally[it.k] != 0) != SMALLY) return;
  nodal_tile<SMALLY, true>(a, it.tile, it.k, make_int2(it.lo, it.hi), a.part_ws + (size_t)i * (size_t)(64 * RTX_SC_ROWS));
}

__global__ __launch_bounds__(256) void split_combine_kernel(ScArgs a) {
  constexpr int TILE = 64 * RTX_SC_ROWS;
  const int i = blockIdx.x;
  if (i >= *a.n_items) return;
  const SplitItem it = a.items[i];
  if (it.part != 1) return;
  const long long ia = (long long)it.tile * TILE;
  for (int t = threadIdx.x; t < TILE; t += 256) {
    const long long p = ia + t;
    if (p >= a.g.n) break;
    const size_t o = (size_t)it.k * (size_t)a.ld + (size_t)p;
    float v = a.out32 ? a.out32[o] : 0.f;
    double v64 = a.out64 ? a.out64[o] : 0.0;
    for (int e = 0; e < it.extra; ++e) {
      const float w = a.part_ws[(size_t)(i + e) * TILE + t];
      v += w;
      v64 += (double)w * a.inv_scale;
    }
    if (a.out32) a.out32[o] = v;
    if (a.out64) a.out64[o] = v64;
  }
}

__attribute__((visibility("hidden"))) int rtx_voigt_scatter_tile_points(void) { return 64 * RTX_SC_ROWS; }

int rtx_voigt_sum_scatter(const rtx_prep* P, const rtx_grid* grid, int n_layers, float* out_f32, double* out_f64, int64_t ld,
                          hipStream_t st, void (*launch_ranges)(const rtx_prep*, const rtx_grid*, int, int, int, hipStream_t, int),
                          int nodal) {
  constexpr int TILE = 64 * RTX_SC_ROWS;
  const long long n_tiles_ll = (grid->n + TILE - 1) / TILE;
  if (n_tiles_ll > P->max_tiles) RTX_FAIL("grid shard of %lld points exceeds the prep capacity", (long long)grid->n);
  const int n_tiles = (int)n_tiles_ll;
  if (nodal && P->split_bound > 0 && P->items.get()) RTX_HIP(hipMemsetAsync(P->n_items, 0, sizeof(int), st));
  launch_ranges(P, grid, n_layers, n_tiles, TILE, st, nodal);
  RTX_LAUNCH_CHECK();
  ScArgs a;
  a.rec = P->rec.get(); a.rec64 = P->rec64.get(); a.ranges = P->ranges.get(); a.smally = P->smally; a.n_lines = P->n_lines;
  a.n_tiles = n_tiles; a.tiles_per_xcd = xcd_slots(n_tiles);
  a.g = to_dev(grid);
  a.out32 = out_f32; a.out64 = out_f64; a.ld = ld; a.inv_scale = 1.0 / P->scale;
  a.stamp = nullptr;
  a.items = P->items.get(); a.n_items = P->n_items; a.part_ws = P->part_ws.get();
#if RTX_SC_STAMP
  static unsigned long long* d_stamp = nullptr;
  static size_t stamp_cap = 0;
  const size_t n_stamp = (size_t)8 * a.tiles_per_xcd * n_layers * SC_NW * SC_NSTAMP;
  if (stamp_cap < n_stamp) {
    if (d_stamp) RTX_HIP(hipFree(d_stamp));
    RTX_HIP(hipMalloc(&d_stamp, n_stamp * sizeof(unsigned long long)));
    stamp_cap = n_stamp;
  }
  RTX_HIP(hipMemsetAsync(d_stamp, 0, n_stamp * sizeof(unsigned long long), st));
  a.stamp = d_stamp;
#endif
  static int lds_pad = -1;
  if (lds_pad < 0) { const char* e = getenv("RADTXFR_DEBUG_LDS_PAD"); lds_pad = e ? atoi(e) : 0; }
  if (nodal) {
    hipLaunchKernelGGL((voigt_nodal_kernel<false>), dim3(8 * a.tiles_per_xcd, n_layers), dim3(64 * SC_NW), (size_t)lds_pad, st, a);
    RTX_LAUNCH_CHECK();
    hipLaunchKernelGGL((voigt_nodal_kernel<true>), dim3(8 * ((a.tiles_per_xcd + 15) / 16), n_layers), dim3(64 * SC_NW), 0, st, a);
    if (P->split_bound > 0 && P->items.get()) {
      RTX_LAUNCH_CHECK();
      const unsigned cap = (unsigned)P->split_bound;
      hipLaunchKernelGGL((voigt_nodal_parts_kernel<false>), dim3(cap), dim3(64 * SC_NW), 0, st, a);
      hipLaunchKernelGGL((voigt_nodal_parts_kernel<true>), dim3(cap), dim3(64 * SC_NW), 0, st, a);
      hipLaunchKernelGGL(split_combine_kernel, dim3(cap), dim3(256), 0, st, a);
    }
  } else {
    hipLaunchKernelGGL((voigt_scatter_kernel<false>), dim3(8 * a.tiles_per_xcd, n_layers), dim3(256), 0, st, a);
  }
  RTX_LAUNCH_CHECK();
#if RTX_SC_STAMP
  {
    std::vector<unsigned long long> hbuf(n_stamp);
    RTX_HIP(hipMemcpyAsync(hbuf.data(), d_stamp, n_stamp * sizeof(unsigned long long), hipMemcpyDeviceToHost, st));
    RTX_HIP(hipStreamSynchronize(st));
    if (const char* fn = getenv("RADTXFR_STAMP_FILE")) {
      FILE* fh = fopen(fn, "wb");
      if (fh) { fwrite(hbuf.data(), sizeof(unsigned long long), n_stamp, fh); fclose(fh); }
    }
    double h[SC_NSTAMP] = {0};
    for (size_t i = 0; i < n_stamp; ++i) h[i % SC_NSTAMP] += (double)hbuf[i];
    const double w = (double)SC_NW * 8 * a.tiles_per_xcd * n_layers;
    fprintf(stderr, "[stamp] per wave (s_memtime ticks): load+geom %.0f emit %.0f rowlevel %.0f entry %.0f pp %.0f band %.0f barrier %.0f life %.0f\n",
            h[0] / w, h[1] / w, h[2] / w, h[3] / w, h[4] / w, h[5] / w, h[6] / w, h[7] / w);
  }
#endif
  if (!nodal) {
    hipLaunchKernelGGL((voigt_scatter_kernel<true>), dim3(8 * ((a.tiles_per_xcd + 15) / 16), n_layers), dim3(256), 0, st, a);
    RTX_LAUNCH_CHECK();
  }
  return 0;
}
```

### radtxfr_amd/engine.py

```python
import ctypes as C
from typing import NamedTuple, Optional

import numpy as np
import torch

from . import _lib, tips

TUD_MAX_MU = 8
TUD_OD_NONNEG = 1

CBOLTS = 1.380648813e-16
TREF = 296.0


def volumeConcentration(p, T):
    return (p / 9.869233e-7) / (CBOLTS * T)


class trace_range:
    enabled = bool(int(__import__("os").environ.get("RADTXFR_ROCTX", "0") or 0))

    def __init__(self, name):
        self.name = name

    def __enter__(self):
        if trace_range.enabled:
            torch.cuda.nvtx.range_push(self.name)

    def __exit__(self, *exc):
        if trace_range.enabled:
            torch.cuda.nvtx.range_pop()
        return False


def require_gpu():
    if not torch.cuda.is_available():
        raise _lib.RtxError("no HIP device visible: radtxfr_amd has no CPU fallback (torch.cuda.is_available() is False)")


def device(dev=None):
    require_gpu()
    if dev is None:
        return torch.device("cuda", torch.cuda.current_device())
    return torch.device(dev)


def _stream_ptr():
    return C.c_void_p(torch.cuda.current_stream().cuda_stream)


def _ptr(t):
    return C.c_void_p(t.data_ptr()) if t is not None else C.c_void_p(0)


def _h(a):
    a = np.ascontiguousarray(a, dtype=np.float64)
    return a, a.ctypes.data_as(C.c_void_p)


class Grid:

    def __init__(self, xmin, xmax, n_total, offset=0, n=None):
        self.c = _lib.make_grid(xmin, xmax, n_total, offset, n)

    xmin = property(lambda s: s.c.xmin)
    xmax = property(lambda s: s.c.xmax)
    step = property(lambda s: s.c.step)
    n_total = property(lambda s: s.c.n_total)
    offset = property(lambda s: s.c.offset)
    n = property(lambda s: s.c.n)

    def shard(self, offset, n):
        return Grid(self.xmin, self.xmax, self.n_total, offset, n)

    def axis(self):
        ig = np.arange(self.offset, self.offset + self.n, dtype=np.float64)
        X = ig * self.step + self.xmin
        if self.n and self.offset + self.n == self.n_total:
            X[-1] = self.xmax
        return X

    def x_at(self, i):
        ig = self.offset + int(i)
        return self.xmax if ig == self.n_total - 1 else float(np.float64(ig) * self.step + self.xmin)

    @staticmethod
    def from_axis(X, rtol=1e-9):
        X = np.asarray(X, dtype=np.float64).ravel()
        if X.size < 2:
            raise ValueError("spectral axis needs at least 2 points")
        g = Grid(X[0], X[-1], X.size)
        dev = np.max(np.abs(X - np.linspace(X[0], X[-1], X.size)))
# ... 608 lines not shown
    nn = np.array([a[2] for a in axes], dtype=np.int32)
    vp = C.c_void_p
    _lib.check(_lib.load().rtx_continuum_add_d(grid.byref(), nL, T.ctypes.data_as(vp), len(axes), v0.ctypes.data_as(vp),
                                               dv.ctypes.data_as(vp), nn.ctypes.data_as(vp), A.ctypes.data_as(vp),
                                               A_T.ctypes.data_as(vp), A_x.ctypes.data_as(vp), A.shape[2], slots.ctypes.data_as(vp),
                                               len(species) if K is not None else 0, _ptr(dOD_dT), _ptr(K), lds[0], _stream_ptr(), 0))
    return dOD_dT, K


class TudGeometry(NamedTuple):
    Z_s: np.ndarray
    mu: np.ndarray
    mask: np.ndarray
    n_down: int


def tud_geometry(Z, Altitudes, theta_r):
    Z = np.atleast_1d(np.asarray(Z, dtype=np.float64))
    Z_s = np.array([Altitudes], dtype=np.float64).ravel()
    mu = np.ascontiguousarray(np.array([1.0 / np.cos(np.asarray(theta_r, dtype=np.float64))], dtype=np.float64).ravel())
    mask = np.ascontiguousarray(np.stack([(Z <= zs) for zs in Z_s]).astype(np.uint8))
    n_down = int(mask[-1].sum())
    return TudGeometry(Z_s, mu, mask, n_down)


def _check_tud_outputs(tau, Lu, Ld, nrow, n):
    for t in (tau, Lu):
        assert t.dtype == torch.float32 and t.is_cuda and t.dim() == 2 and t.shape[0] == nrow
        assert t.shape[1] >= n and t.stride(1) == 1 and t.stride(0) == tau.stride(0)
    assert Ld.dtype == torch.float32 and Ld.is_cuda and Ld.numel() >= n and Ld.stride(0) == 1
    return tau.stride(0) if tau.shape[0] > 1 else max(tau.shape[1], n)


def tud(OD, grid, T, Z, Altitudes=(500,), theta_r=0.0, N_angle=30, returnOD=False, per_angle=False, out=None,
        od_nonneg=False):
    lib = _lib.load()
    T = np.atleast_1d(np.asarray(T, dtype=np.float64))
    Z_s, mu_s, mask, n_down = tud_geometry(Z, Altitudes, theta_r)
    nL = T.size
    assert OD.dtype == torch.float32 and OD.is_cuda and OD.dim() == 2 and OD.shape[0] == nL and OD.shape[1] >= grid.n
    assert OD.stride(1) == 1
    if mu_s.size > TUD_MAX_MU:
        if out is not None:
            raise ValueError("engine.tud: out= is limited to %d slant paths per call" % TUD_MAX_MU)
        th = np.asarray(theta_r, dtype=np.float64).ravel()
        tau = torch.empty((Z_s.size, mu_s.size, grid.n), dtype=torch.float32, device=OD.device)
        Lu = torch.empty_like(tau)
        Ld_ang = None
        for m0 in range(0, mu_s.size, TUD_MAX_MU):
            m1 = min(m0 + TUD_MAX_MU, mu_s.size)
            res = tud(OD, grid, T, Z, Altitudes=Altitudes, theta_r=th[m0:m1], N_angle=N_angle, returnOD=returnOD,
                      per_angle=per_angle and m0 == 0, od_nonneg=od_nonneg)
            t_c, l_c, Ld_c = res[:3]
            if m0 == 0:
                Ld = Ld_c
                Ld_ang = res[4] if per_angle else None
            tau[:, m0:m1] = t_c.view(Z_s.size, m1 - m0, grid.n)
            Lu[:, m0:m1] = l_c.view(Z_s.size, m1 - m0, grid.n)
        if per_angle:
            return tau.view(-1, grid.n), Lu.view(-1, grid.n), Ld, (Z_s.size, mu_s.size), Ld_ang
        return tau.view(-1, grid.n), Lu.view(-1, grid.n), Ld, (Z_s.size, mu_s.size)
    dev = OD.device
    if out is None:
        tau = torch.empty((Z_s.size * mu_s.size, grid.n), dtype=torch.float32, device=dev)
        Lu = torch.empty_like(tau)
        Ld = torch.empty((grid.n,), dtype=torch.float32, device=dev)
    else:
        tau, Lu, Ld = out
    ld_out = _check_tud_outputs(tau, Lu, Ld, Z_s.size * mu_s.size, grid.n)
    Ld_ang = torch.empty((int(N_angle), ld_out), dtype=torch.float32, device=dev) if per_angle else None
    T_h, T_p = _h(T)
    mu_h, mu_p = _h(mu_s)
    _lib.check(lib.rtx_tud_opts(_ptr(OD), OD.stride(0), grid.byref(), nL, T_p, Z_s.size, mask.ctypes.data_as(C.c_void_p),
                                mu_s.size, mu_p, n_down, int(N_angle), int(bool(returnOD)), _ptr(tau), _ptr(Lu), _ptr(Ld),
                                _ptr(Ld_ang), ld_out, _stream_ptr(), TUD_OD_NONNEG if od_nonneg else 0))
    if per_angle:
        return tau, Lu, Ld, (Z_s.size, mu_s.size), Ld_ang[:, :grid.n]
    return tau, Lu, Ld, (Z_s.size, mu_s.size)


class TudRunner:

    def __init__(self, lines, grid, Z, n_layers=None, Altitudes=(500,), theta_r=0.0, N_angle=30, returnOD=False, out=None,
                 OD=None, plan=None, broadening=None, xs_lut=None, continuum=None):
        self.lib = _lib.load()
        self.lines, self.grid = lines, grid
        self.continuum = continuum
        self.foreign = broadening_gases(broadening)
        self.xs_lut = xs_lut
        if xs_lut is not None:
            if broadening is not None:
                raise NotImplementedError("xs_lut with broadening=%r: a table's broadening was fixed when it was made" % (broadening,))
            self._xs_off = xs_lut.align(grid) + grid.offset
        Z = np.atleast_1d(np.asarray(Z, dtype=np.float64))
        self.nL = int(Z.size if n_layers is None else n_layers)
        Z_s, self.mu, self.mask, self.n_down = tud_geometry(Z, Altitudes, theta_r)
        if self.mu.size > TUD_MAX_MU:
            raise ValueError("TudRunner takes at most %d slant paths" % TUD_MAX_MU)
        self.shape = (Z_s.size, self.mu.size)
        self.N_angle, self.returnOD = int(N_angle), int(bool(returnOD))
        dev = device()
        nrow = Z_s.size * self.mu.size
        self.OD = OD if OD is not None else torch.empty((self.nL, grid.n), dtype=torch.float32, device=dev)
        if out is None:
            self.tau = torch.empty((nrow, grid.n), dtype=torch.float32, device=dev)
            self.Lu = torch.empty_like(self.tau)
            self.Ld = torch.empty((grid.n,), dtype=torch.float32, device=dev)
        else:
            self.tau, self.Lu, self.Ld = out
        self.set_outputs(self.tau, self.Lu, self.Ld)
        if xs_lut is not None:
            self.plan = None
            if OD is None:
                self.OD = torch.empty((self.nL, (grid.n + 3) // 4 * 4), dtype=torch.float32, device=dev)[:, :grid.n]
            return
        self.plan = plan if plan is not None else lines.plan(self.nL, grid.n)
        self._env = np.empty(2 * self.nL + 2 * len(lines.species) * self.nL + len(lines.species), dtype=np.float64)

    def set_outputs(self, tau, Lu, Ld):
        self._ld_out = _check_tud_outputs(tau, Lu, Ld, self.shape[0] * self.shape[1], self.grid.n)
        self.tau, self.Lu, self.Ld = tau, Lu, Ld
        self._ptrs = (C.c_void_p(tau.data_ptr()), C.c_void_p(Lu.data_ptr()), C.c_void_p(Ld.data_ptr()))

    def _add_continuum(self, T, P_pa, PL_km, MF_VAL, MF_ID, st):
        tables, axes = self.continuum.layer_tables(T, P_pa, PL_km, MF_VAL, MF_ID)
        _continuum_call(self.lib, tables, axes, self.grid, T, self.OD, st)

    def run(self, T, P_pa, PL_km, MF_VAL, MF_ID, partitionFunction=None):
        nL, lines = self.nL, self.lines
        T = np.ascontiguousarray(T, dtype=np.float64)
        assert T.size == nL
        if self.xs_lut is not None:
            vp, st = C.c_void_p, _stream_ptr()
            rows, wx = self.xs_lut.layer_terms(T, np.asarray(P_pa, dtype=np.float64) / 101325.0, PL_km, MF_VAL, MF_ID)
            with trace_range("rtx_xs_od + rtx_tud"):
                _lib.check(self.lib.rtx_xs_od(self.xs_lut._handle(), self._xs_off, self.grid.n, nL, rows.ctypes.data_as(vp),
                                              wx.ctypes.data_as(vp), vp(self.OD.data_ptr()), self.OD.stride(0), st))
                if self.continuum is not None:
                    self._add_continuum(T, P_pa, PL_km, MF_VAL, MF_ID, st)
                _lib.check(self.lib.rtx_tud(
                    vp(self.OD.data_ptr()), self.OD.stride(0), self.grid.byref(), nL, T.ctypes.data_as(vp), self.shape[0],
                    self.mask.ctypes.data_as(vp), self.shape[1], self.mu.ctypes.data_as(vp), self.n_down, self.N_angle, self.returnOD,
                    self._ptrs[0], self._ptrs[1], self._ptrs[2], None, self._ld_out, st))
            return self.tau, self.Lu, self.Ld
        w, p_atm = layer_weights_od(lines.species, T, P_pa, PL_km, MF_VAL, MF_ID)
        qratio, mass = species_factors(lines.species, T, partitionFunction, weight=w)
        nS = len(lines.species)
        env = self._env
        env[0:nL] = T
        env[nL:2 * nL] = p_atm
        env[2 * nL:2 * nL + nS * nL] = qratio.ravel()
        env[2 * nL + nS * nL:2 * nL + 2 * nS * nL] = w.ravel()
        env[2 * nL + 2 * nS * nL:] = mass
        base = env.ctypes.data
        vp = C.c_void_p
        if self.foreign is not None:
            dil = broadening_fractions(lines.species, np.asarray(MF_VAL, dtype=np.float64).reshape(nL, -1), MF_ID, self.foreign)
            st = _stream_ptr()
            with trace_range("rtx_line_prep_mix + rtx_voigt_sum + rtx_tud"):
                _line_prep(None, self.lib.rtx_line_prep_mix,
                           (self.plan._h, lines._h, self.grid.byref(), nL, vp(base), vp(base + 8 * nL), vp(base + 16 * nL),
                            vp(base + 8 * (2 * nL + nS * nL)), vp(base + 8 * (2 * nL + 2 * nS * nL))),
                           lines, nL, dil, None, None, 0.0, 50.0, 0.0, 1.0, 0, st)
                _lib.check(self.lib.rtx_voigt_sum(self.plan._h, self.grid.byref(), nL, vp(self.OD.data_ptr()), None,
                                                  self.OD.stride(0), st))
                if self.continuum is not None:
                    self._add_continuum(T, P_pa, PL_km, MF_VAL, MF_ID, st)
                _lib.check(self.lib.rtx_tud(
                    vp(self.OD.data_ptr()), self.OD.stride(0), self.grid.byref(), nL, vp(base), self.shape[0],
                    self.mask.ctypes.data_as(vp), self.shape[1], self.mu.ctypes.data_as(vp), self.n_down, self.N_angle, self.returnOD,
                    self._ptrs[0], self._ptrs[1], self._ptrs[2], None, self._ld_out, st))
            return self.tau, self.Lu, self.Ld
        if self.continuum is not None:
            st = _stream_ptr()
            nonneg = TUD_OD_NONNEG if bool(np.all(np.isfinite(env)) and env.min() >= 0.0) else 0
            with trace_range("rtx_line_prep + rtx_voigt_sum + rtx_continuum_add + rtx_tud"):
                _lib.check(self.lib.rtx_line_prep(
                    self.plan._h, lines._h, self.grid.byref(), nL, vp(base), vp(base + 8 * nL), vp(base + 16 * nL),
                    vp(base + 8 * (2 * nL + nS * nL)), vp(base + 8 * (2 * nL + 2 * nS * nL)), 1.0, 0.0, 0.0, 50.0, 0.0, 1.0, st))
                _lib.check(self.lib.rtx_voigt_sum(self.plan._h, self.grid.byref(), nL, vp(self.OD.data_ptr()), None,
                                                  self.OD.stride(0), st))
                self._add_continuum(T, P_pa, PL_km, MF_VAL, MF_ID, st)
                _lib.check(self.lib.rtx_tud_opts(
                    vp(self.OD.data_ptr()), self.OD.stride(0), self.grid.byref(), nL, vp(base), self.shape[0],
                    self.mask.ctypes.data_as(vp), self.shape[1], self.mu.ctypes.data_as(vp), self.n_down, self.N_angle, self.returnOD,
                    self._ptrs[0], self._ptrs[1], self._ptrs[2], None, self._ld_out, st, nonneg))
            return self.tau, self.Lu, self.Ld
        with trace_range("rtx_compute_tud"):
            _lib.check(self.lib.rtx_compute_tud(
                self.plan._h, lines._h, self.grid.byref(), nL, vp(base), vp(base + 8 * nL), vp(base + 16 * nL),
                vp(base + 8 * (2 * nL + nS * nL)), vp(base + 8 * (2 * nL + 2 * nS * nL)), 1.0, 0.0, 0.0, 50.0, 0.0,
                self.shape[0], self.mask.ctypes.data_as(vp), self.shape[1], self.mu.ctypes.data_as(vp), self.n_down, self.N_angle,
                self.returnOD, vp(self.OD.data_ptr()), self.OD.stride(0), self._ptrs[0], self._ptrs[1], self._ptrs[2], self._ld_out,
                _stream_ptr()))
        return self.tau, self.Lu, self.Ld


class TudPipelines:

    def __init__(self, lines, grid, Z, n_layers=None, n_pipes=2, outs=None, **kw):
        self.streams = [torch.cuda.Stream() for _ in range(int(n_pipes))]
        self.runs = []
        nL = int(np.atleast_1d(Z).size if n_layers is None else n_layers)
        for p, s in enumerate(self.streams):
            with torch.cuda.stream(s):
                self.runs.append(TudRunner(lines, grid, Z, n_layers=nL, plan=VoigtPlan(lines, nL, grid.n),
                                           out=None if outs is None else outs[p], **kw))
        self.k = 0

    def run(self, T, P_pa, PL_km, MF_VAL, MF_ID):
        p = self.k % len(self.runs)
        self.k += 1
        with torch.cuda.stream(self.streams[p]):
            out = self.runs[p].run(T, P_pa, PL_km, MF_VAL, MF_ID)
        return p, out

    def close(self):
        torch.cuda.synchronize()
        for r in self.runs:
            r.plan.close()
        self.runs = []


def planck(X, T, wavelength=False, grid=None):
    lib = _lib.load()
    nx = grid.n if X is None else X.numel()
    out = torch.empty((nx, T.numel()), dtype=torch.float64, device=T.device)
    _lib.check(lib.rtx_planck(grid.byref() if grid is not None else None, _ptr(X), nx, _ptr(T), T.numel(),
                              int(bool(wavelength)), _ptr(out), _stream_ptr()))
    return out


def apparent_radiance(X, emis, Ts, tau, La, Ld, dT=None, return_Ls=False):
    lib = _lib.load()
    nX, nE = emis.shape
    nA = Ts.numel()
    nT = dT.numel() if dT is not None else 1
    L = torch.empty((nX, nE, nA, nT), dtype=torch.float32, device=emis.device)
    Ls = torch.empty_like(L) if return_Ls else None
    if L.numel() == 0:
        return L, Ls
    _lib.check(lib.rtx_apparent_radiance(_ptr(X), nX, _ptr(emis), nE, _ptr(Ts), nA, _ptr(tau), _ptr(La), _ptr(Ld),
                                         _ptr(dT), nT if dT is not None else 0, _ptr(L), _ptr(Ls), _stream_ptr()))
    return L, Ls


def ils(kind, Y, centre, sigma, X=None, grid=None):
    lib = _lib.load()
    assert Y.dtype == torch.float32 and Y.is_cuda and Y.dim() == 2 and Y.stride(1) == 1
    nx, nS = Y.shape
    nB = centre.numel()
    out = torch.empty((nB, nS), dtype=torch.float32, device=Y.device)
    _lib.check(lib.rtx_ils(int(kind), grid.byref() if grid is not None else None, _ptr(X), nx, _ptr(Y), nS, Y.stride(0),
                           nB, _ptr(centre), _ptr(sigma), _ptr(out), _stream_ptr()))
    return out


def max_wing_cm(columns, T_layers, p_atm_layers, omega_wing=0.0, omega_wing_hw=50.0):
    T = np.asarray(T_layers, dtype=np.float64)
    p = np.asarray(p_atm_layers, dtype=np.float64)
    nu = np.asarray(columns["nu"], dtype=np.float64)
    if nu.size == 0:
        return float(omega_wing)
    g = float(np.max(columns["gamma_air"]))
    n_hi, n_lo = float(np.max(columns["n_air"])), float(np.min(columns["n_air"]))
    tr = TREF / T
    g0 = g * np.max(p * np.maximum(tr ** n_hi, tr ** n_lo))
    gd = 3.6e-7 * float(np.max(nu)) * np.sqrt(float(np.max(T)) / 1.0)
    shift = float(np.max(np.abs(columns["delta_air"]))) * float(np.max(p))
    return max(float(omega_wing), omega_wing_hw * g0, omega_wing_hw * min(gd, 10.0 * g0 + 1.0)) + shift


TILE_COST = {"tile": 100.0, "reach": 30.0, "centre": 0.0, "band_row": 24.0}


def tile_costs(columns, xmin, step, n_total, T_layers, p_atm_layers, tile, omega_wing=0.0, omega_wing_hw=50.0, coef=None):
    c = dict(TILE_COST)
# ... 306 lines not shown
        key = [species[s] for s in use]
        out[use] = -tips.partition_sums_dT(key, T_layers) / tips.partition_sums(key, T_layers)
    return out


def voigt_sum_dT(lines, grid, T, p_atm, weight, out_f32=None, dlnw_dT=None, out_f64=None, dil_air=1.0, dil_self=0.0,
                 omega_wing=0.0, omega_wing_hw=50.0, intensity_threshold=0.0, scale=1.0, qratio=None, mass=None, dlnq_dT=None):
    lib = _lib.load()
    if not isinstance(grid, Grid):
        raise TypeError("voigt_sum_dT: a uniform Grid is required (explicit axes are not supported)")
    if qratio is not None and dlnq_dT is None:
        raise ValueError("voigt_sum_dT: a caller's qratio needs its dlnq_dT")
    nL, env = _prologue_inputs(lines, T, p_atm, weight, None, qratio, mass)
    T_a = env[0][0]
    nS = len(lines.species)
    if dlnq_dT is None:
        dlnq_dT = species_dlnq_dT(lines.species, T_a, weight=weight)
    if dlnw_dT is None:
        dlnw_dT = -1.0 / T_a
    dlnsw = np.ascontiguousarray(np.broadcast_to(np.asarray(dlnq_dT, dtype=np.float64), (nS, nL))
                                 + np.broadcast_to(np.asarray(dlnw_dT, dtype=np.float64), (nS, nL)))
    plan = lines.plan(nL, grid.n)
    st = _stream_ptr()
    _lib.check(lib.rtx_line_prep_dt(plan._h, lines._h, grid.byref(), nL, *(e[1] for e in env), dlnsw.ctypes.data_as(C.c_void_p),
                                    float(dil_air), float(dil_self), float(omega_wing), float(omega_wing_hw),
                                    float(intensity_threshold), float(scale), st))
    _check_outputs(nL, grid.n, out_f32, out_f64)
    _lib.check(lib.rtx_voigt_sum_dt(plan._h, grid.byref(), nL, _ptr(out_f32), _ptr(out_f64), grid.n, st))
    return out_f32, out_f64


def jacobian_species_columns(MF_ID, wrt):
    ids = [int(v) for v in np.asarray(MF_ID).ravel()]
    cols = []
    for w in wrt:
        if isinstance(w, str):
            continue
        if int(w) not in ids:
            raise ValueError("wrt: molecule id %r is not in MFs_ID %r" % (w, ids))
        cols.append(ids.index(int(w)))
    return cols


class JacobianStages(NamedTuple):
    T: np.ndarray
    Z: np.ndarray
    layers: np.ndarray
    t_pos: int
    tau: torch.Tensor
    Lu: torch.Tensor
    Ld: torch.Tensor
    OD: torch.Tensor
    OD_plus: Optional[torch.Tensor]
    OD_minus: Optional[torch.Tensor]
    dOD_dT: Optional[torch.Tensor]
    K: Optional[torch.Tensor]


def _jacobian_stages(what, lines, grid, Z, T, P_pa, PL_km, MF_VAL, MF_ID, Altitudes, theta_r, N_angle, returnOD, wrt, layers,
                     fd_step_T, mark, dT_method="fd", continuum=None, xs_lut=None):
    check_dT_method(dT_method)
    T = np.ascontiguousarray(np.atleast_1d(np.asarray(T, dtype=np.float64)))
    Z = np.atleast_1d(np.asarray(Z, dtype=np.float64))
    nL = T.size
    P_pa = np.atleast_1d(np.asarray(P_pa, dtype=np.float64))
    PL_km = np.atleast_1d(np.asarray(PL_km, dtype=np.float64))
    MF_VAL = np.asarray(MF_VAL, dtype=np.float64).reshape(nL, -1)
    wrt = tuple(wrt)
    if len(set(wrt)) != len(wrt) or any(isinstance(w_, str) and w_ != "T" for w_ in wrt):
        raise ValueError("wrt: distinct entries, each \"T\" or a molecule id of MFs_ID (got %r)" % (wrt,))
    with_T = "T" in wrt
    spec_cols = jacobian_species_columns(MF_ID, wrt)
    layers = np.arange(nL, dtype=np.int32) if layers is None else np.ascontiguousarray(np.asarray(layers, dtype=np.int32).ravel())
    if layers.size == 0 or layers.min() < 0 or layers.max() >= nL:
        raise ValueError("layers: indices must lie in [0, %d)" % nL)
    if with_T and dT_method == "fd" and not (fd_step_T > 0.0):
        raise ValueError("fd_step_T must be > 0")
    th = np.asarray(theta_r, dtype=np.float64).ravel()
    if th.size != 1:
        raise NotImplementedError("%s: one slant path (theta_r) per call" % what)
    jacobian_limits(nL, np.array([Altitudes]).size, N_angle, len(spec_cols))
    dev = device()
    run = TudRunner(lines, grid, Z, n_layers=nL, Altitudes=Altitudes, theta_r=theta_r, N_angle=N_angle, returnOD=returnOD,
                    continuum=continuum, xs_lut=xs_lut)
    tau, Lu, Ld = run.run(T, P_pa, PL_km, MF_VAL, MF_ID)
    OD = run.OD
    if mark:
        mark("base")
    n = grid.n
    ODp = ODm = dOD = None
    if xs_lut is not None:
        return _xs_jacobian_columns(xs_lut, grid, Z, T, P_pa, PL_km, MF_VAL, MF_ID, wrt, layers, fd_step_T, mark, dT_method, continuum,
                                    tau, Lu, Ld, OD)
    if with_T and dT_method == "analytic":
        dOD = torch.empty((nL, n), dtype=torch.float32, device=dev)
        w, p_atm = layer_weights_od(lines.species, T, P_pa, PL_km, MF_VAL, MF_ID)
        voigt_sum_dT(lines, grid, T, p_atm, w, dOD)
    elif with_T:
        ODp = torch.empty((nL, n), dtype=torch.float32, device=dev)
        ODm = torch.empty_like(ODp)
        for sgn, out in ((1.0, ODp), (-1.0, ODm)):
            Ts = T + sgn * float(fd_step_T)
            w, p_atm = layer_weights_od(lines.species, Ts, P_pa, PL_km, MF_VAL, MF_ID)
            voigt_sum_window(lines, grid, Ts, T, p_atm, w, out)
            if continuum is not None:
                continuum_add(continuum, grid, Ts, P_pa, PL_km, MF_VAL, MF_ID, out)
    if mark:
        mark("T")
    K = None
    if spec_cols:
        K = torch.empty((len(spec_cols), nL, n), dtype=torch.float32, device=dev)
        for s, c in enumerate(spec_cols):
            unit = np.zeros_like(MF_VAL)
            unit[:, c] = 1.0
            w, p_atm = layer_weights_od(lines.species, T, P_pa, PL_km, unit, MF_ID)
            voigt_sum(lines, grid, T, p_atm, w, out_f32=K[s])
    if continuum is not None and (dOD is not None or K is not None):
        continuum_add_d(continuum, grid, T, P_pa, PL_km, MF_VAL, MF_ID, dOD_dT=dOD, K=K,
                        species=[w_ for w_ in wrt if not isinstance(w_, str)])
    if mark:
        mark("species")
    t_pos = wrt.index("T") if with_T else 0
    return JacobianStages(T, Z, layers, t_pos, tau, Lu, Ld, OD, ODp, ODm, dOD, K)


def _xs_jacobian_columns(lut, grid, Z, T, P_pa, PL_km, MF_VAL, MF_ID, wrt, layers, fd_step_T, mark, dT_method, continuum, tau, Lu, Ld, OD):
    nL, n, ld, dev = T.size, grid.n, OD.stride(0), OD.device
    with_T = "T" in wrt
    species = [w_ for w_ in wrt if not isinstance(w_, str)]
    P_atm = P_pa / 101325.0
    column = lambda: torch.empty((nL, ld), dtype=torch.float32, device=dev)[:, :n]
    ODp = ODm = dOD = K = None
    if with_T and dT_method == "analytic":
        dOD = column()
    elif with_T:
        ODp, ODm = column(), column()
        for sgn, out in ((1.0, ODp), (-1.0, ODm)):
            Ts = T + sgn * float(fd_step_T)
            xs_od(lut, grid, Ts, P_atm, PL_km, MF_VAL, MF_ID, out_f32=out)
            if continuum is not None:
                continuum_add(continuum, grid, Ts, P_pa, PL_km, MF_VAL, MF_ID, out)
    if species:
        K = torch.empty((len(species), nL, ld), dtype=torch.float32, device=dev)[:, :, :n]
    if dOD is not None or K is not None:
        xs_od_d(lut, grid, T, P_atm, PL_km, MF_VAL, MF_ID, dOD_dT=dOD, K=K, species=species)
    if mark:
        mark("T")
    if continuum is not None and (dOD is not None or K is not None):
        continuum_add_d(continuum, grid, T, P_pa, PL_km, MF_VAL, MF_ID, dOD_dT=dOD, K=K, species=species)
    if mark:
        mark("species")
    return JacobianStages(T, Z, layers, wrt.index("T") if with_T else 0, tau, Lu, Ld, OD, ODp, ODm, dOD, K)


def tud_jacobian(lines, grid, Z, T, P_pa, PL_km, MF_VAL, MF_ID, Altitudes=(500,), theta_r=0.0, N_angle=30, returnOD=False,
                 wrt=("T",), layers=None, fd_step_T=0.5, block_bytes=JAC_BLOCK_BYTES, on_block=None, mark=None, dT_method="fd",
                 continuum=None, xs_lut=None):
    s = _jacobian_stages("tud_jacobian", lines, grid, Z, T, P_pa, PL_km, MF_VAL, MF_ID, Altitudes, theta_r, N_angle, returnOD, wrt,
                         layers, fd_step_T, mark, dT_method, continuum, xs_lut)
    J = tud_jacobian_from_od(s.OD, s.OD_plus, s.OD_minus, fd_step_T, s.K, s.tau, grid, s.T, s.Z, Altitudes=Altitudes,
                             theta_r=theta_r, N_angle=N_angle, returnOD=returnOD, layers=s.layers, t_pos=s.t_pos,
                             block_bytes=block_bytes, on_block=on_block, mark=mark, dOD_dT=s.dOD_dT)
    return s.tau, s.Lu, s.Ld, s.OD, J


class _JacobianFront(NamedTuple):
    entry: object
# ... 204 lines not shown
```

### radtxfr_amd/radiative_transfer.py

```python
import functools
import os
import threading
import time

import numpy as np
import torch

from . import _hostio, engine
from . import hapi as _hapi

c1 = 1.19104295315e-16
c2 = 1.43877736830e-02

_CSV = os.path.join(os.path.dirname(os.path.abspath(__file__)), "data", "StandardAtmosphere.csv")
StdAtmosCSV = np.loadtxt(_CSV, delimiter=",", skiprows=1)
StdAtmos = StdAtmosCSV.copy()
StdAtmos[:, 1:6] = np.round(StdAtmosCSV[:, 1:6], 2)
StdAtmos[:, 6:] = np.vectorize(lambda v: float("%.3E" % v))(StdAtmosCSV[:, 6:])

options = {
    "DVOUT": 0.0005,
    "T": 296.0, "P": 101325.0, "PL": 1.0,
    "MF_ID": np.array([]), "MF_VAL": np.array([]),
    "line_table": None,
# ... 156 lines not shown
    def __init__(self, fn, Xmin, Xmax, opts, kwargs):
        self.fn, self.Xmin, self.Xmax = fn, Xmin, Xmax
        self.o = o = dict(opts)
        o.update(kwargs)
        self.Z, self.T, self.P, self.PL, self.MF = (np.asarray(o[k], dtype=np.float64) for k in ("Zs", "Ts", "Ps", "PLs", "MFs_VAL"))
        self.ID = np.asarray(o["MFs_ID"])
        self.Z_s = np.array([o["Altitudes"]]).ravel()
        self.theta = np.asarray(o["theta_r"], dtype=np.float64)
        self.N_angle, self.returnOD = int(o["N_angle"]), bool(o["returnOD"])
        self.broadening = o.get("broadening")

    lut = functools.cached_property(lambda self: _xs_lut_option(self.fn, self.o))
    continuum = functools.cached_property(lambda self: _continuum_option(self.fn, self.o, self.ID))
    foreign = functools.cached_property(lambda self: engine.broadening_gases(self.broadening))
    X = functools.cached_property(lambda self: _cached_axis(self.Xmin, self.Xmax, self.o["DVOUT"]))
    grid = functools.cached_property(lambda self: engine.Grid(self.Xmin, self.Xmax, self.X.size))

    def table(self):
        return _resolve_table(self.o.get("line_table"), self.foreign or ()) if self.lut is None else None


_STAGING = {}
_TRACE = float(os.environ.get("RADTXFR_TRACE", "0") or 0)


def _rows_to_host_f64(rows, stream=None):
    got = _hostio.rows_to_pinned_f64(rows, stream)
    if got is not None:
        return got
    key = (rows[0].device.index, threading.get_ident())
    st = _STAGING.get(key)
    if st is None:
        st = _STAGING[key] = _hostio.Staging(depth=1)
    ticket = st.stage(rows, stream)
    return st.collect(ticket), ticket[3]


def _tud_shapes(tau2, Lu2, nZ, nMu):
    tau_ = tau2.reshape(nZ, nMu, -1).transpose(2, 0, 1)
    Lu_ = Lu2.reshape(nZ, nMu, -1).transpose(2, 0, 1)
    if nZ == 1 and nMu == 1:
        return tau_[:, 0, 0], Lu_[:, 0, 0]
    if nZ == 1:
        return np.ascontiguousarray(tau_[:, 0, :]), np.ascontiguousarray(Lu_[:, 0, :])
    if nMu == 1:
        return np.ascontiguousarray(tau_[:, :, 0]), np.ascontiguousarray(Lu_[:, :, 0])
    return np.ascontiguousarray(tau_), np.ascontiguousarray(Lu_)


_SIDE_STREAMS = {}


def _compute_tud_chunked(tbl, grid, Z, T, P, PL, MF, ID, Z_s, theta, nA, returnOD, n_chunks, broadening=None, xs_lut=None,
                         continuum=None):
    from . import _lib, dist as _dist
    n = grid.n
    tile = int(_lib.load().rtx_voigt_tile_points())
    offs = _dist.tile_aligned_bounds(n, n_chunks, tile)
    nL = T.size
    nZ, nMu = Z_s.size, np.atleast_1d(theta).size
    nrow = nZ * nMu
    lent = _hostio.lend_block((2 * nrow + 1, n))
    if lent is None:
        return None
    host, arr = lent
    dev = engine.device()
    tau = torch.empty((nrow, n), dtype=torch.float32, device=dev)
    Lu = torch.empty_like(tau)
    Ld = torch.empty((n,), dtype=torch.float32, device=dev)
    max_len = int(np.diff(offs).max())
    OD = torch.empty((nL, max_len), dtype=torch.float32, device=dev)
    plan = tbl.plan(nL, n) if xs_lut is None else None
    side = _SIDE_STREAMS.get(dev.index)
    if side is None:
        side = _SIDE_STREAMS[dev.index] = torch.cuda.Stream()
    done = None
    for c in range(n_chunks):
        off, ln = int(offs[c]), int(offs[c + 1] - offs[c])
        if ln == 0:
            continue
        sl = slice(off, off + ln)
        run = engine.TudRunner(tbl, grid.shard(grid.offset + off, ln), Z, n_layers=nL, Altitudes=Z_s, theta_r=theta, N_angle=nA,
                               returnOD=returnOD, out=(tau[:, sl], Lu[:, sl], Ld[sl]), OD=OD[:, :ln], plan=plan,
                               broadening=broadening, xs_lut=xs_lut, continuum=continuum)
        run.run(T, P, PL, MF, ID)
        ready = torch.cuda.Event()
        ready.record()
        with torch.cuda.stream(side):
            side.wait_event(ready)
            blk = torch.empty((2 * nrow + 1, ln), dtype=torch.float64, device=dev)
            blk[:nrow].copy_(tau[:, sl])
            blk[nrow:2 * nrow].copy_(Lu[:, sl])
            blk[2 * nrow].copy_(Ld[sl])
            for r in range(2 * nrow + 1):
                host[r, sl].copy_(blk[r], non_blocking=True)
            done = torch.cuda.Event()
            done.record(side)
    for t in (tau, Lu, Ld, OD):
        t.record_stream(side)
    if done is not None:
        done.synchronize()
    return arr[:nrow], arr[nrow:2 * nrow], arr[2 * nrow:], (nZ, nMu)


def compute_TUD(Xmin, Xmax, opts=options, **kwargs):
    trace = [time.perf_counter()] if _TRACE else None
    c = _Call("compute_TUD", Xmin, Xmax, opts, kwargs)
    o, lut, broadening, cont = c.o, c.lut, c.broadening, c.continuum
    Z, T, P, PL, MF, ID, Z_s, nA = c.Z, c.T, c.P, c.PL, c.MF, c.ID, c.Z_s, c.N_angle
    X_, grid = c.X, c.grid
    if trace:
        trace.append(time.perf_counter())
    tbl = c.table()
    if trace:
        trace.append(time.perf_counter())
    if o.get("copy_axis"):
        X_ = _hostio.copy_threaded(X_)
    chunks = o.get("chunks")
    if chunks is None:
        chunks = 4 if grid.n >= 2000000 else 2 if grid.n >= 500000 else 1
    if chunks > 1 and c.theta.size <= engine.TUD_MAX_MU and not o["save"]:
        got = _compute_tud_chunked(tbl, grid, Z, T, P, PL, MF, ID, Z_s, c.theta, nA, c.returnOD, int(chunks), broadening=broadening,
                                   xs_lut=lut, continuum=cont)
        if got is not None:
            tau_h, Lu_h, Ld_h, (nZ, nMu) = got
            if trace:
                trace.append(time.perf_counter())
                if trace[-1] - trace[0] > _TRACE * 1e-3:
                    print("compute_TUD %.1f ms (chunked x%d): options+axis %.2f  table %.2f  kernels + copies %.2f"
                          % tuple([1e3 * (trace[-1] - trace[0]), chunks] + [1e3 * (b - a) for a, b in zip(trace, trace[1:])]), flush=True)
            tau_, Lu_ = _tud_shapes(tau_h, Lu_h, nZ, nMu)
            return X_, tau_, Lu_, Ld_h[0]
    if c.theta.size <= engine.TUD_MAX_MU and not o["save"]:
        run = engine.TudRunner(tbl, grid, Z, n_layers=T.size, Altitudes=Z_s, theta_r=c.theta, N_angle=nA, returnOD=c.returnOD,
                               broadening=broadening, xs_lut=lut, continuum=cont)
        tau, Lu, Ld = run.run(T, P, PL, MF, ID)
        nZ, nMu = run.shape
        OD = run.OD
    else:
        if lut is not None:
            OD = engine.xs_od(lut, grid, T, P / 101325.0, PL, MF, ID)
        else:
            OD = engine.optical_depths(tbl, grid, T, P, PL, MF, ID, broadening=broadening)
        if cont is not None:
            engine.continuum_add(cont, grid, T, P, PL, MF, ID, OD)
        res = engine.tud(OD, grid, T, Z, Altitudes=Z_s, theta_r=c.theta, N_angle=nA, returnOD=c.returnOD, per_angle=bool(o["save"]))
        tau, Lu, Ld, (nZ, nMu) = res[:4]
    if trace:
        trace.append(time.perf_counter())
    (tau_h, Lu_h, Ld_h), done = _rows_to_host_f64([tau, Lu, Ld[None, :]])
    if trace:
        trace.append(time.perf_counter())
    done.synchronize()
    if trace:
        trace.append(time.perf_counter())
        if trace[-1] - trace[0] > _TRACE * 1e-3:
            print("compute_TUD %.1f ms: options+axis %.2f  table %.2f  enqueue kernels %.2f  enqueue copies %.2f  wait %.2f"
                  % tuple(1e3 * v for v in [trace[-1] - trace[0]] + [b - a for a, b in zip(trace, trace[1:])]), flush=True)
    tau_, Lu_ = _tud_shapes(tau_h, Lu_h, nZ, nMu)
    Ld_ = Ld_h[0]
    if o["save"]:
        angles = np.linspace(0, np.pi / 2.0, nA, endpoint=False)
        t3 = tau_h.reshape(nZ, nMu, -1).transpose(2, 0, 1)
        u3 = Lu_h.reshape(nZ, nMu, -1).transpose(2, 0, 1)
        np.savez("ComputeTUD.npz", OD=OD.double().cpu().numpy().T, B=planckian(X_, T), tau=t3, Ld=res[4].double().cpu().numpy().T,
                 Lu=u3, X=X_, angles=angles, Z_s=Z_s, mu_s=np.array([1.0 / np.cos(o["theta_r"])]).ravel())
    return X_, tau_, Lu_, Ld_
# ... 775 lines not shown
```

Measured before the change: 111.2 billion wavenumber*layer points/s.

## Split Voigt OD and TUD into two passes to skip opaque middle layers

```diff
diff --git a/include/radtxfr_hip.h b/include/radtxfr_hip.h
--- a/include/radtxfr_hip.h
+++ b/include/radtxfr_hip.h
@@ -146,6 +146,14 @@
                     const uint8_t* mask_h, int n_mu, const double* mu_h, int n_down, int n_angle,
                     int return_od, float* OD, int64_t ld_od, float* tau, float* Lu, float* Ld,
                     int64_t ld_out, void* stream);
+#define RTX_CTUD_OD_SCRATCH 1u
+int rtx_compute_tud_opts(rtx_prep* prep, const rtx_lines* lines, const rtx_grid* grid, int n_layers,
+                         const double* T_h, const double* p_atm_h, const double* qratio_h,
+                         const double* weight_h, const double* mass_h, double dil_air, double dil_self,
+                         double omega_wing, double omega_wing_hw, double intensity_threshold, int n_alt,
+                         const uint8_t* mask_h, int n_mu, const double* mu_h, int n_down, int n_angle,
+                         int return_od, float* OD, int64_t ld_od, float* tau, float* Lu, float* Ld,
+                         int64_t ld_out, void* stream, unsigned flags);
 
 int rtx_apparent_radiance(const double* X, int64_t nX, const float* emis, int64_t nE,
                           const double* Ts, int64_t nA, const float* tau, const float* La,
diff --git a/radtxfr_amd/_lib.py b/radtxfr_amd/_lib.py
--- a/radtxfr_amd/_lib.py
+++ b/radtxfr_amd/_lib.py
@@ -61,6 +61,8 @@
     "rtx_tud_gtable": (_i32, [_i32, _vp, _vp]),
     "rtx_compute_tud": (_i32, [_vp, _vp, _gp, _i32, _vp, _vp, _vp, _vp, _vp, _dbl, _dbl, _dbl, _dbl, _dbl, _i32, _vp, _i32, _vp,
                                 _i32, _i32, _i32, _vp, _i64, _vp, _vp, _vp, _i64, _vp]),
+    "rtx_compute_tud_opts": (_i32, [_vp, _vp, _gp, _i32, _vp, _vp, _vp, _vp, _vp, _dbl, _dbl, _dbl, _dbl, _dbl, _i32, _vp, _i32, _vp,
+                                     _i32, _i32, _i32, _vp, _i64, _vp, _vp, _vp, _i64, _vp, C.c_uint]),
     "rtx_apparent_radiance": (_i32, [_vp, _i64, _vp, _i64, _vp, _i64, _vp, _vp, _vp, _vp, _i64, _vp, _vp, _vp]),
     "rtx_ils": (_i32, [_i32, _gp, _vp, _i64, _vp, _i64, _i64, _i32, _vp, _vp, _vp, _vp]),
     "rtx_srf_apply": (_i32, [_gp, _vp, _i64, _vp, _i64, _i64, _i32, _vp, _vp, _vp, _vp, _vp, _vp]),
diff --git a/radtxfr_amd/csrc/rtx_common.h b/radtxfr_amd/csrc/rtx_common.h
--- a/radtxfr_amd/csrc/rtx_common.h
+++ b/radtxfr_amd/csrc/rtx_common.h
@@ -175,4 +175,14 @@
   DevBuf<LineRecDT64> drec64;
   DevBuf<double> dlnsw;
   int dT = 0;
+  DevBuf<unsigned char> done;
 };
+
+struct VoigtLayers {
+  int n_a, k_a, k_b, n_y;
+  const unsigned char* done;
+  bool ranges;
+};
+__attribute__((visibility("hidden"))) bool rtx_voigt_layers_ok(const rtx_prep* P);
+__attribute__((visibility("hidden"))) int rtx_voigt_sum_layers(const rtx_prep* P, const rtx_grid* grid, int n_layers, float* out_f32,
+                                                                int64_t ld, void* stream, const VoigtLayers& sel);
diff --git a/radtxfr_amd/csrc/rtx_tud.hip b/radtxfr_amd/csrc/rtx_tud.hip
--- a/radtxfr_amd/csrc/rtx_tud.hip
+++ b/radtxfr_amd/csrc/rtx_tud.hip
@@ -153,6 +153,8 @@
   const double* gtab;
   double g0;
   int skip;
+  unsigned char* done;
+  float early_smin;
 };
 
 #define TUD_OPAQUE_Y 26.0f
@@ -560,11 +562,32 @@
 #define TUD_SKIP_MARGIN 8.0f
 #define TUD_SKIP_TAU0 151.0f
 
-template <bool PN, bool SKIP>
+template <bool PN, bool SKIP, int PHASE = 0>
 __global__ __launch_bounds__(256) void tud_g_kernel(TudArgs a) {
   static_assert(PN || !SKIP, "the look at the top is written for the Planck-node instantiation");
+  static_assert(PHASE == 0 || SKIP, "the two-launch pass belongs to the instantiation that may look");
   __shared__ double s_g[TUDG_NINT * 8];
   __shared__ float s_stage[(SKIP ? 2 : 1) * TUD_STAGE][256];
+  unsigned done4 = 0u;
+  if (PHASE == 2) {
+    done4 = reinterpret_cast<const unsigned*>(a.done)[blockIdx.x];
+    if (done4 == 0x01010101u) return;
+  }
+  if (PHASE == 1) {
+    __shared__ int s_may[4];
+    const long long i_pre = (long long)blockIdx.x * blockDim.x + threadIdx.x;
+    const float* __restrict__ od_pre = a.OD + (i_pre < a.g.n ? i_pre : a.g.n - 1);
+    float s_pre = 0.f;
+#pragma unroll
+    for (int t = 0; t < TUD_STAGE; ++t) s_pre += od_pre[(size_t)(t < a.n_layers ? t : a.n_layers - 1) * a.ld];
+    const bool may = __ballot(s_pre >= a.early_smin) == ~0ull;
+    if ((threadIdx.x & 63) == 0) s_may[threadIdx.x >> 6] = may ? 1 : 0;
+    __syncthreads();
+    if (!(s_may[0] | s_may[1] | s_may[2] | s_may[3])) {
+      if ((threadIdx.x & 63) == 0) a.done[(size_t)blockIdx.x * 4 + (threadIdx.x >> 6)] = 0;
+      return;
+    }
+  }
   tudg_load(s_g, a);
   TudLane ln(a);
   const int nL = a.n_layers;
@@ -577,6 +600,10 @@
   PlanckNodes PNd;
   if (PN) PNd = planck_nodes_setup(a, ln);
   __syncthreads();
+  if (PHASE == 2 && ((done4 >> (8 * (threadIdx.x >> 6))) & 1u)) return;
+  auto not_done = [&]() {
+    if ((threadIdx.x & 63) == 0) a.done[(size_t)blockIdx.x * 4 + (threadIdx.x >> 6)] = 0;
+  };
 
   for (int p = 1; p < a.n_alt * a.n_mu; ++p) {
     const int ia = p / a.n_mu, im = p - ia * a.n_mu;
@@ -656,7 +683,9 @@
         if (k_hi <= TUD_SKIP_BOTTOM && k_hi + TUD_STAGE <= k_top) { k_look = k_hi; break; }
       }
     }
-  }
+    if (PHASE == 1) break;
+  }
+  if (PHASE == 1 && k_look < 0) { not_done(); return; }
   if (SKIP && k_look >= 0) {
     int kc = k_look;
     unsigned tid_top = threadIdx.x;
@@ -696,6 +725,10 @@
 #pragma unroll
       for (int t = TUD_STAGE - 1; t >= 0; --t) s_top += s_stage[slot + t][threadIdx.x];
       if (__ballot(s_top * ac0 >= y_up) == ~0ull) k_res = k_top - c * TUD_STAGE;
+    }
+    if (PHASE == 1) {
+      if (k_res < 0 || (kc < k_res && __ballot((s0 + s_top) * ac0 >= TUD_SKIP_TAU0) != ~0ull)) { not_done(); return; }
+      if ((threadIdx.x & 63) == 0) a.done[(size_t)blockIdx.x * 4 + (threadIdx.x >> 6)] = 1;
     }
     if (k_res < 0) {
 #pragma unroll
@@ -993,6 +1026,27 @@
   return 0;
 }
 
+static float tudg_early_smin(int n_angle) {
+  static std::mutex mu;
+  static std::map<int, float> memo;
+  std::lock_guard<std::mutex> lock(mu);
+  auto it = memo.find(n_angle);
+  if (it != memo.end()) return it->second;
+  const TudQuadrature quad = tud_quadrature(n_angle);
+  float r = -INFINITY;
+  if (n_angle > 1 && quad.wsum > 0.0) {
+    auto G = [&](double S) { double g = 0.0; for (int ii = 1; ii < n_angle; ++ii) g += quad.w[ii] * exp(-S / cos(quad.th[ii])); return g; };
+    const double target = quad.wsum * exp2(-26.5);
+    double lo = 0.0, hi = TUDG_SMAX;
+    if (G(hi) < target) {
+      for (int it2 = 0; it2 < 60; ++it2) { const double mid = 0.5 * (lo + hi); (G(mid) > target ? lo : hi) = mid; }
+      r = (float)(lo * (1.0 - 1e-4));
+    }
+  }
+  memo[n_angle] = r;
+  return r;
+}
+
 static int tudg_table(int n_angle, DevTableCache<double>::Hit* out) {
   static DevTableCache<double>* const cache = new DevTableCache<double>(0);
   int dev = 0;
@@ -1018,9 +1072,25 @@
   return tud_launch(tud_kernel<NA, false>, a, (size_t)TUD_STAGE * 256 * sizeof(float), st);
 }
 
-extern "C" int rtx_tud_opts(const float* OD, int64_t ld, const rtx_grid* grid, int n_layers, const double* T_h, int n_alt,
-                            const uint8_t* mask_h, int n_mu, const double* mu_h, int n_down, int n_angle, int return_od,
-                            float* tau, float* Lu, float* Ld, float* Ld_angles, int64_t ld_out, void* stream, unsigned flags) {
+static bool tud_force_streams() {
+  static int v = -1;
+  if (v < 0) { const char* e = getenv("RADTXFR_TUD_KERNEL"); v = (e && !strcmp(e, "streams")) ? 1 : 0; }
+  return v != 0;
+}
+static bool tud_skip_on() {
+  static int v = -1;
+  if (v < 0) { const char* e = getenv("RADTXFR_TUD_SKIP"); v = (e && !strcmp(e, "0")) ? 0 : 1; }
+  return v != 0;
+}
+static bool tud_planck_nodes(const rtx_grid* grid, double t_min) {
+  const double nu_lo = grid->xmin;
+  return nu_lo > 0.0 && (4.0 / nu_lo + RT_C2 * 100.0 / t_min) * 63.0 * grid->step <= 7e-3;
+}
+
+static int tud_opts_impl(const float* OD, int64_t ld, const rtx_grid* grid, int n_layers, const double* T_h, int n_alt,
+                         const uint8_t* mask_h, int n_mu, const double* mu_h, int n_down, int n_angle, int return_od,
+                         float* tau, float* Lu, float* Ld, float* Ld_angles, int64_t ld_out, void* stream, unsigned flags,
+                         int phase, unsigned char* done) {
   if (rtx_check_grid(grid)) return 1;
   if (flags & ~(unsigned)RTX_TUD_OD_NONNEG) RTX_FAIL("flags=0x%x: unknown bits", flags);
   if (!OD || !T_h || !mask_h || !mu_h || !tau || !Lu || !Ld) RTX_FAIL("a required pointer is NULL");
@@ -1062,8 +1132,8 @@
   a.inv_wsum = (float)(1.0 / quad.wsum);
   if (na == 0) a.inv_wsum = NAN;
   hipStream_t st = (hipStream_t)stream;
-  static int force_streams = -1;
-  if (force_streams < 0) { const char* e = getenv("RADTXFR_TUD_KERNEL"); force_streams = (e && !strcmp(e, "streams")) ? 1 : 0; }
+  const bool force_streams = tud_force_streams();
+  if (phase != 0 && (Ld_angles || force_streams)) RTX_FAIL("internal: a two-launch pass without tud_g_kernel");
   if (!Ld_angles && !force_streams) {
     DevTableCache<double>::Hit gt;
     if (tudg_table(n_angle, &gt)) return 1;
@@ -1072,15 +1142,19 @@
     for (int ia = 0; ia < n_alt && prefix; ++ia)
       for (int k = 0; k < n_layers; ++k)
         if ((mask_h[(size_t)ia * n_layers + k] != 0) != (k < a.count[ia])) { prefix = false; break; }
-    const double nu_lo = grid->xmin;
-    const bool pn = nu_lo > 0.0 && (4.0 / nu_lo + RT_C2 * 100.0 / t_min) * 63.0 * grid->step <= 7e-3;
+    const bool pn = tud_planck_nodes(grid, t_min);
     void (*kernel)(TudArgs);
+    if (phase != 0 && n_alt * n_mu != 1) RTX_FAIL("internal: a two-launch pass with more than one pair");
     if (n_alt * n_mu == 1) {
       kernel = pn ? tud_g_kernel<true, false> : tud_g_kernel<false, false>;
-      static int skip_on = -1;
-      if (skip_on < 0) { const char* e = getenv("RADTXFR_TUD_SKIP"); skip_on = (e && !strcmp(e, "0")) ? 0 : 1; }
-      a.skip = skip_on && (flags & RTX_TUD_OD_NONNEG) && !return_od && prefix && pn;
+      a.skip = tud_skip_on() && (flags & RTX_TUD_OD_NONNEG) && !return_od && prefix && pn;
       if (a.skip) kernel = tud_g_kernel<true, true>;
+      if (phase != 0) {
+        if (!a.skip || !done) RTX_FAIL("internal: a two-launch pass without the look at the top");
+        a.done = done;
+        a.early_smin = n_down >= TUD_STAGE ? tudg_early_smin(n_angle) : -INFINITY;
+        kernel = phase == 1 ? tud_g_kernel<true, true, 1> : tud_g_kernel<true, true, 2>;
+      }
     }
     else if (prefix && n_mu == 1) kernel = pn ? tud_g_snap_kernel<1, true> : tud_g_snap_kernel<1, false>;
     else if (prefix) kernel = pn ? tud_g_snap_kernel<TUD_MAX_MU, true> : tud_g_snap_kernel<TUD_MAX_MU, false>;
@@ -1095,11 +1169,84 @@
   return launch_tud<32>(a, na, st);
 }
 
+extern "C" int rtx_tud_opts(const float* OD, int64_t ld, const rtx_grid* grid, int n_layers, const double* T_h, int n_alt,
+                            const uint8_t* mask_h, int n_mu, const double* mu_h, int n_down, int n_angle, int return_od,
+                            float* tau, float* Lu, float* Ld, float* Ld_angles, int64_t ld_out, void* stream, unsigned flags) {
+  return tud_opts_impl(OD, ld, grid, n_layers, T_h, n_alt, mask_h, n_mu, mu_h, n_down, n_angle, return_od, tau, Lu, Ld, Ld_angles,
+                       ld_out, stream, flags, 0, nullptr);
+}
+
 extern "C" int rtx_tud(const float* OD, int64_t ld, const rtx_grid* grid, int n_layers, const double* T_h, int n_alt,
                        const uint8_t* mask_h, int n_mu, const double* mu_h, int n_down, int n_angle, int return_od,
                        float* tau, float* Lu, float* Ld, float* Ld_angles, int64_t ld_out, void* stream) {
   return rtx_tud_opts(OD, ld, grid, n_layers, T_h, n_alt, mask_h, n_mu, mu_h, n_down, n_angle, return_od, tau, Lu, Ld, Ld_angles,
                       ld_out, stream, 0u);
+}
+
+static bool tud_split_layers(const rtx_grid* grid, int n_layers, const double* T_h, int n_alt, const uint8_t* mask_h, int n_mu,
+                             int return_od, unsigned tud_flags, int* k_mid0, int* k_mid1) {
+  if (!tud_skip_on() || tud_force_streams() || !(tud_flags & RTX_TUD_OD_NONNEG) || return_od) return false;
+  if (!grid || !T_h || !mask_h || n_alt != 1 || n_mu != 1 || n_layers < 1 || n_layers > TUD_MAX_LAYERS) return false;
+  int cnt0 = 0;
+  for (int k = 0; k < n_layers; ++k) cnt0 += mask_h[k] != 0;
+  for (int k = 0; k < n_layers; ++k)
+    if ((mask_h[k] != 0) != (k < cnt0)) return false;
+  double t_min = T_h[0];
+  for (int k = 1; k < n_layers; ++k) t_min = T_h[k] < t_min ? T_h[k] : t_min;
+  if (!tud_planck_nodes(grid, t_min)) return false;
+  if (cnt0 < 1) return false;
+  const int k_top = (cnt0 - 1) & ~(TUD_STAGE - 1);
+  const int k_deep = k_top - (TUD_SKIP_SCAN - TUD_STAGE);
+  if (TUD_SKIP_BOTTOM + TUD_STAGE > k_deep) return false;
+  *k_mid0 = TUD_SKIP_BOTTOM; *k_mid1 = k_deep;
+  return true;
+}
+
+static bool od_skip_on() {
+  static int v = -1;
+  if (v < 0) { const char* e = getenv("RADTXFR_OD_SKIP"); v = (e && !strcmp(e, "0")) ? 0 : 1; }
+  return v != 0;
+}
+
+extern "C" int rtx_compute_tud_opts(rtx_prep* prep, const rtx_lines* lines, const rtx_grid* grid, int n_layers, const double* T_h,
+                                    const double* p_atm_h, const double* qratio_h, const double* weight_h, const double* mass_h,
+                                    double dil_air, double dil_self, double omega_wing, double omega_wing_hw,
+                                    double intensity_threshold, int n_alt, const uint8_t* mask_h, int n_mu, const double* mu_h,
+                                    int n_down, int n_angle, int return_od, float* OD, int64_t ld_od, float* tau, float* Lu,
+                                    float* Ld, int64_t ld_out, void* stream, unsigned flags) {
+  if (flags & ~(unsigned)RTX_CTUD_OD_SCRATCH) RTX_FAIL("flags=0x%x: unknown bits", flags);
+  if (!OD) RTX_FAIL("OD workspace is NULL");
+  if (rtx_line_prep_profile(prep, lines, grid, n_layers, T_h, p_atm_h, qratio_h, weight_h, mass_h, dil_air, dil_self, omega_wing,
+                            omega_wing_hw, intensity_threshold, 1.0, RTX_PROFILE_VOIGT, stream))
+    return 1;
+  auto nonneg = [](const double* v, long long n) {
+    for (long long j = 0; j < n; ++j)
+      if (!(v[j] >= 0.0 && v[j] <= 1.7976931348623157e308)) return false;
+    return true;
+  };
+  const long long n_sl = (long long)lines->n_species * n_layers;
+  const unsigned tud_flags = nonneg(weight_h, n_sl) && nonneg(qratio_h, n_sl) && nonneg(T_h, n_layers) && nonneg(p_atm_h, n_layers)
+                                 ? RTX_TUD_OD_NONNEG : 0u;
+  int k_mid0 = 0, k_mid1 = 0;
+  if ((flags & RTX_CTUD_OD_SCRATCH) && od_skip_on() && grid->n > 0 && rtx_voigt_layers_ok(prep) &&
+      tud_split_layers(grid, n_layers, T_h, n_alt, mask_h, n_mu, return_od, tud_flags, &k_mid0, &k_mid1)) {
+    const size_t n_done = (size_t)((grid->n + 1023) / 1024) * 16;
+    if (rtx_voigt_tile_points() != 1024) RTX_FAIL("internal: the done flags are laid out for tiles of 16 rows of 64 points");
+    if (prep->done.reserve(n_done)) return 1;
+    unsigned char* done = prep->done.get();
+    const VoigtLayers la{k_mid0, 0, k_mid1, k_mid0 + (n_layers - k_mid1), nullptr, true};
+    const VoigtLayers lb{k_mid1 - k_mid0, k_mid0, 0, k_mid1 - k_mid0, done, false};
+    if (rtx_voigt_sum_layers(prep, grid, n_layers, OD, ld_od, stream, la)) return 1;
+    if (tud_opts_impl(OD, ld_od, grid, n_layers, T_h, n_alt, mask_h, n_mu, mu_h, n_down, n_angle, return_od, tau, Lu, Ld, nullptr,
+                      ld_out, stream, tud_flags, 1, done))
+      return 1;
+    if (rtx_voigt_sum_layers(prep, grid, n_layers, OD, ld_od, stream, lb)) return 1;
+    return tud_opts_impl(OD, ld_od, grid, n_layers, T_h, n_alt, mask_h, n_mu, mu_h, n_down, n_angle, return_od, tau, Lu, Ld, nullptr,
+                         ld_out, stream, tud_flags, 2, done);
+  }
+  if (rtx_voigt_sum(prep, grid, n_layers, OD, nullptr, ld_od, stream)) return 1;
+  return rtx_tud_opts(OD, ld_od, grid, n_layers, T_h, n_alt, mask_h, n_mu, mu_h, n_down, n_angle, return_od, tau, Lu, Ld, nullptr,
+                      ld_out, stream, tud_flags);
 }
 
 extern "C" int rtx_compute_tud(rtx_prep* prep, const rtx_lines* lines, const rtx_grid* grid, int n_layers, const double* T_h,
@@ -1108,19 +1255,7 @@
                                double intensity_threshold, int n_alt, const uint8_t* mask_h, int n_mu, const double* mu_h,
                                int n_down, int n_angle, int return_od, float* OD, int64_t ld_od, float* tau, float* Lu,
                                float* Ld, int64_t ld_out, void* stream) {
-  if (!OD) RTX_FAIL("OD workspace is NULL");
-  if (rtx_line_prep_profile(prep, lines, grid, n_layers, T_h, p_atm_h, qratio_h, weight_h, mass_h, dil_air, dil_self, omega_wing,
-                            omega_wing_hw, intensity_threshold, 1.0, RTX_PROFILE_VOIGT, stream))
-    return 1;
-  if (rtx_voigt_sum(prep, grid, n_layers, OD, nullptr, ld_od, stream)) return 1;
-  auto nonneg = [](const double* v, long long n) {
-    for (long long j = 0; j < n; ++j)
-      if (!(v[j] >= 0.0 && v[j] <= 1.7976931348623157e308)) return false;
-    return true;
-  };
-  const long long n_sl = (long long)lines->n_species * n_layers;
-  const unsigned flags = nonneg(weight_h, n_sl) && nonneg(qratio_h, n_sl) && nonneg(T_h, n_layers) && nonneg(p_atm_h, n_layers)
-                             ? RTX_TUD_OD_NONNEG : 0u;
-  return rtx_tud_opts(OD, ld_od, grid, n_layers, T_h, n_alt, mask_h, n_mu, mu_h, n_down, n_angle, return_od, tau, Lu, Ld, nullptr,
-                      ld_out, stream, flags);
-}
+  return rtx_compute_tud_opts(prep, lines, grid, n_layers, T_h, p_atm_h, qratio_h, weight_h, mass_h, dil_air, dil_self, omega_wing,
+                              omega_wing_hw, intensity_threshold, n_alt, mask_h, n_mu, mu_h, n_down, n_angle, return_od, OD, ld_od,
+                              tau, Lu, Ld, ld_out, stream, 0u);
+}
diff --git a/radtxfr_amd/csrc/rtx_voigt.hip b/radtxfr_amd/csrc/rtx_voigt.hip
--- a/radtxfr_amd/csrc/rtx_voigt.hip
+++ b/radtxfr_amd/csrc/rtx_voigt.hip
@@ -106,7 +106,7 @@
 
 int rtx_voigt_sum_scatter(const rtx_prep* P, const rtx_grid* grid, int n_layers, float* out_f32, double* out_f64, int64_t ld,
                           hipStream_t st, void (*launch_ranges)(const rtx_prep*, const rtx_grid*, int, int, int, hipStream_t, int),
-                          int nodal);
+                          int nodal, const VoigtLayers* sel = nullptr);
 
 static void launch_tile_ranges(const rtx_prep* P, const rtx_grid* grid, int n_layers, int n_tiles, int tile, hipStream_t st, int split) {
   RangeArgs ra;
@@ -153,3 +153,20 @@
   }
   return rtx_voigt_sum_scatter(P, grid, n_layers, out_f32, out_f64, ld, st, launch_tile_ranges, voigt_kernel_choice() == 0);
 }
+
+bool rtx_voigt_layers_ok(const rtx_prep* P) {
+  return P && !P->axis && P->n_lines > 0 && voigt_kernel_choice() == 0 && !(P->split_bound > 0 && P->items.get());
+}
+int rtx_voigt_sum_layers(const rtx_prep* P, const rtx_grid* grid, int n_layers, float* out_f32, int64_t ld, void* stream,
+                         const VoigtLayers& sel) {
+  if (!rtx_voigt_layers_ok(P)) RTX_FAIL("internal: a layer subset on a prologue that cannot take one");
+  if (rtx_check_grid(grid)) return 1;
+  if (n_layers < 1 || n_layers != P->n_layers) RTX_FAIL("n_layers=%d does not match the last rtx_line_prep (%d)", n_layers, P->n_layers);
+  if (!out_f32) RTX_FAIL("the output is NULL");
+  if (ld < grid->n) RTX_FAIL("ld=%lld < n=%lld", (long long)ld, (long long)grid->n);
+  if (sel.n_a < 0 || sel.n_y < sel.n_a || sel.n_y < 1 || sel.k_a < 0 || sel.k_a + sel.n_a > n_layers || sel.k_b < 0 ||
+      sel.k_b + (sel.n_y - sel.n_a) > n_layers)
+    RTX_FAIL("internal: layer subset outside [0,%d)", n_layers);
+  if (grid->n == 0) return 0;
+  return rtx_voigt_sum_scatter(P, grid, n_layers, out_f32, nullptr, ld, (hipStream_t)stream, launch_tile_ranges, 1, &sel);
+}
diff --git a/radtxfr_amd/csrc/rtx_voigt_scatter.hip b/radtxfr_amd/csrc/rtx_voigt_scatter.hip
--- a/radtxfr_amd/csrc/rtx_voigt_scatter.hip
+++ b/radtxfr_amd/csrc/rtx_voigt_scatter.hip
@@ -50,7 +50,22 @@
   const SplitItem* items;
   const int* n_items;
   float* part_ws;
+  int n_a, k_a, k_b;
+  const unsigned char* done;
 };
+__device__ __forceinline__ int sc_layer(const ScArgs& a, int y) { return y < a.n_a ? a.k_a + y : a.k_b + (y - a.n_a); }
+__device__ __forceinline__ unsigned sc_done_rows(const ScArgs& a, int b) {
+  static_assert(RTX_SC_ROWS == 16, "a tile's done flags are read as four dwords");
+  const int tile = xcd_tile(b);
+  if (!a.done || tile >= a.n_tiles) return 0u;
+  const uint4 d = reinterpret_cast<const uint4*>(a.done)[tile];
+  auto nib = [](unsigned w) -> unsigned { return (((w & 0x01010101u) * 0x01020408u) >> 24) & 0xFu; };
+  unsigned m = nib(d.x) | (nib(d.y) << 4) | (nib(d.z) << 8) | (nib(d.w) << 12);
+  const long long left = a.g.n - (long long)tile * (64 * RTX_SC_ROWS);
+  const int rows_in = left >= 64 * RTX_SC_ROWS ? RTX_SC_ROWS : (int)((left + 63) >> 6);
+  m |= (0xFFFFu << rows_in) & 0xFFFFu;
+  return m;
+}
 
 struct RowGeom {
   int r_lo, r_hi;
@@ -336,7 +351,7 @@
 #endif
 template <bool SMALLY, bool PARTS = false>
 __device__ __forceinline__ void nodal_tile(const ScArgs& a, const int b_or_tile, const int k, const int2 part_rng = make_int2(0, 0),
-                                           float* __restrict__ part_out = nullptr) {
+                                           float* __restrict__ part_out = nullptr, const unsigned done_rows = 0u) {
   constexpr int ROWS = RTX_SC_ROWS;
   constexpr int TILE = 64 * ROWS;
   __shared__ float s_acc[SC_NW][TILE];
@@ -404,6 +419,9 @@
       const unsigned w0 = (unsigned)__builtin_amdgcn_readfirstlane(__float_as_int(e3.x));
       const unsigned w1 = (unsigned)__builtin_amdgcn_readfirstlane(__float_as_int(e3.y));
       unsigned m_pp = w0 & 0xffffu, m_ed = w0 >> 16, m_bd = w1 & 0xffffu, m_cut = w1 >> 16;
+      if (!PARTS) {
+        m_pp &= ~done_rows; m_ed &= ~done_rows;
+      }
       auto slot = [&]() -> int { return __builtin_amdgcn_readfirstlane(__float_as_int(ent[e][3].z)); };
       STAMP(3);
       if (RTX_SC_ABLATE & 4) m_pp = m_ed = 0u;
@@ -738,6 +756,7 @@
     for (int jj = 0; jj < CHEB_N; ++jj) wl[jj] = CHEB_W[lane][jj];
 #pragma unroll 4
     for (int r = wave; r < ROWS; r += SC_NW) {
+      if ((done_rows >> r) & 1u) continue;
       const int t = r * 64 + lane;
       const long long i = (long long)ia + t;
       float f = 0.f;
@@ -770,15 +789,19 @@
 #endif
 template <bool SMALLY>
 __global__ __launch_bounds__(64 * SC_NW, SMALLY ? RTX_SC_WAVES_SMALLY : RTX_SC_WAVES) void voigt_nodal_kernel(ScArgs a) {
-  const int k = blockIdx.y;
+  const int k = sc_layer(a, blockIdx.y);
   if ((a.smally[k] != 0) != SMALLY) return;
   if (SMALLY) {
     for (int b = blockIdx.x; b < 8 * a.tiles_per_xcd; b += gridDim.x) {
-      nodal_tile<true>(a, b, k);
+      const unsigned done_rows = sc_done_rows(a, b);
+      if (done_rows == 0xFFFFu) continue;
+      nodal_tile<true>(a, b, k, make_int2(0, 0), nullptr, done_rows);
       __syncthreads();
     }
   } else {
-    nodal_tile<false>(a, blockIdx.x, k);
+    const unsigned done_rows = sc_done_rows(a, blockIdx.x);
+    if (done_rows == 0xFFFFu) return;
+    nodal_tile<false>(a, blockIdx.x, k, make_int2(0, 0), nullptr, done_rows);
   }
 }
 
@@ -818,14 +841,18 @@
 
 int rtx_voigt_sum_scatter(const rtx_prep* P, const rtx_grid* grid, int n_layers, float* out_f32, double* out_f64, int64_t ld,
                           hipStream_t st, void (*launch_ranges)(const rtx_prep*, const rtx_grid*, int, int, int, hipStream_t, int),
-                          int nodal) {
+                          int nodal, const VoigtLayers* sel) {
   constexpr int TILE = 64 * RTX_SC_ROWS;
   const long long n_tiles_ll = (grid->n + TILE - 1) / TILE;
   if (n_tiles_ll > P->max_tiles) RTX_FAIL("grid shard of %lld points exceeds the prep capacity", (long long)grid->n);
   const int n_tiles = (int)n_tiles_ll;
   if (nodal && P->split_bound > 0 && P->items.get()) RTX_HIP(hipMemsetAsync(P->n_items, 0, sizeof(int), st));
-  launch_ranges(P, grid, n_layers, n_tiles, TILE, st, nodal);
-  RTX_LAUNCH_CHECK();
+  if (sel && !nodal) RTX_FAIL("internal: a layer subset with the point-by-point kernel");
+  if (!sel || sel->ranges) {
+    launch_ranges(P, grid, n_layers, n_tiles, TILE, st, nodal);
+    RTX_LAUNCH_CHECK();
+  }
+  const int n_y = sel ? sel->n_y : n_layers;
   ScArgs a;
   a.rec = P->rec.get(); a.rec64 = P->rec64.get(); a.ranges = P->ranges.get(); a.smally = P->smally; a.n_lines = P->n_lines;
   a.n_tiles = n_tiles; a.tiles_per_xcd = xcd_slots(n_tiles);
@@ -833,6 +860,7 @@
   a.out32 = out_f32; a.out64 = out_f64; a.ld = ld; a.inv_scale = 1.0 / P->scale;
   a.stamp = nullptr;
   a.items = P->items.get(); a.n_items = P->n_items; a.part_ws = P->part_ws.get();
+  a.n_a = sel ? sel->n_a : n_layers; a.k_a = sel ? sel->k_a : 0; a.k_b = sel ? sel->k_b : 0; a.done = sel ? sel->done : nullptr;
 #if RTX_SC_STAMP
   static unsigned long long* d_stamp = nullptr;
   static size_t stamp_cap = 0;
@@ -848,9 +876,9 @@
   static int lds_pad = -1;
   if (lds_pad < 0) { const char* e = getenv("RADTXFR_DEBUG_LDS_PAD"); lds_pad = e ? atoi(e) : 0; }
   if (nodal) {
-    hipLaunchKernelGGL((voigt_nodal_kernel<false>), dim3(8 * a.tiles_per_xcd, n_layers), dim3(64 * SC_NW), (size_t)lds_pad, st, a);
+    hipLaunchKernelGGL((voigt_nodal_kernel<false>), dim3(8 * a.tiles_per_xcd, n_y), dim3(64 * SC_NW), (size_t)lds_pad, st, a);
     RTX_LAUNCH_CHECK();
-    hipLaunchKernelGGL((voigt_nodal_kernel<true>), dim3(8 * ((a.tiles_per_xcd + 15) / 16), n_layers), dim3(64 * SC_NW), 0, st, a);
+    hipLaunchKernelGGL((voigt_nodal_kernel<true>), dim3(8 * ((a.tiles_per_xcd + 15) / 16), n_y), dim3(64 * SC_NW), 0, st, a);
     if (P->split_bound > 0 && P->items.get()) {
       RTX_LAUNCH_CHECK();
       const unsigned cap = (unsigned)P->split_bound;
diff --git a/radtxfr_amd/engine.py b/radtxfr_amd/engine.py
--- a/radtxfr_amd/engine.py
+++ b/radtxfr_amd/engine.py
@@ -8,6 +8,7 @@
 
 TUD_MAX_MU = 8
 TUD_OD_NONNEG = 1
+CTUD_OD_SCRATCH = 1
 
 CBOLTS = 1.380648813e-16
 TREF = 296.0
@@ -782,7 +783,7 @@
 class TudRunner:
 
     def __init__(self, lines, grid, Z, n_layers=None, Altitudes=(500,), theta_r=0.0, N_angle=30, returnOD=False, out=None,
-                 OD=None, plan=None, broadening=None, xs_lut=None, continuum=None):
+                 OD=None, plan=None, broadening=None, xs_lut=None, continuum=None, keep_od=None):
         self.lib = _lib.load()
         self.lines, self.grid = lines, grid
         self.continuum = continuum
@@ -802,6 +803,8 @@
         dev = device()
         nrow = Z_s.size * self.mu.size
         self.OD = OD if OD is not None else torch.empty((self.nL, grid.n), dtype=torch.float32, device=dev)
+        self.keep_od = keep_od
+        self._own_od = None if OD is not None else self.OD
         if out is None:
             self.tau = torch.empty((nrow, grid.n), dtype=torch.float32, device=dev)
             self.Lu = torch.empty_like(self.tau)
@@ -886,13 +889,14 @@
                     self.mask.ctypes.data_as(vp), self.shape[1], self.mu.ctypes.data_as(vp), self.n_down, self.N_angle, self.returnOD,
                     self._ptrs[0], self._ptrs[1], self._ptrs[2], None, self._ld_out, st, nonneg))
             return self.tau, self.Lu, self.Ld
+        scratch = (self.OD is self._own_od) if self.keep_od is None else not self.keep_od
         with trace_range("rtx_compute_tud"):
-            _lib.check(self.lib.rtx_compute_tud(
+            _lib.check(self.lib.rtx_compute_tud_opts(
                 self.plan._h, lines._h, self.grid.byref(), nL, vp(base), vp(base + 8 * nL), vp(base + 16 * nL),
                 vp(base + 8 * (2 * nL + nS * nL)), vp(base + 8 * (2 * nL + 2 * nS * nL)), 1.0, 0.0, 0.0, 50.0, 0.0,
                 self.shape[0], self.mask.ctypes.data_as(vp), self.shape[1], self.mu.ctypes.data_as(vp), self.n_down, self.N_angle,
                 self.returnOD, vp(self.OD.data_ptr()), self.OD.stride(0), self._ptrs[0], self._ptrs[1], self._ptrs[2], self._ld_out,
-                _stream_ptr()))
+                _stream_ptr(), CTUD_OD_SCRATCH if scratch else 0))
         return self.tau, self.Lu, self.Ld
 
 
@@ -1365,7 +1369,7 @@
     jacobian_limits(nL, np.array([Altitudes]).size, N_angle, len(spec_cols))
     dev = device()
     run = TudRunner(lines, grid, Z, n_layers=nL, Altitudes=Altitudes, theta_r=theta_r, N_angle=N_angle, returnOD=returnOD,
-                    continuum=continuum, xs_lut=xs_lut)
+                    continuum=continuum, xs_lut=xs_lut, keep_od=True)
     tau, Lu, Ld = run.run(T, P_pa, PL_km, MF_VAL, MF_ID)
     OD = run.OD
     if mark:
diff --git a/radtxfr_amd/radiative_transfer.py b/radtxfr_amd/radiative_transfer.py
--- a/radtxfr_amd/radiative_transfer.py
+++ b/radtxfr_amd/radiative_transfer.py
@@ -262,7 +262,7 @@
         sl = slice(off, off + ln)
         run = engine.TudRunner(tbl, grid.shard(grid.offset + off, ln), Z, n_layers=nL, Altitudes=Z_s, theta_r=theta, N_angle=nA,
                                returnOD=returnOD, out=(tau[:, sl], Lu[:, sl], Ld[sl]), OD=OD[:, :ln], plan=plan,
-                               broadening=broadening, xs_lut=xs_lut, continuum=continuum)
+                               broadening=broadening, xs_lut=xs_lut, continuum=continuum, keep_od=False)
         run.run(T, P, PL, MF, ID)
         ready = torch.cuda.Event()
         ready.record()
```

Result: faster. 127.2 billion wavenumber*layer points/s (median of 6 runs) (+14.4%).
